# VISION-SJTU/UniDefense

Measured on AMD Instinct MI355X. Metric: images/sec fwd+bwd (256x256, EffNet-b4), higher is better.
Workload: dtype f32

## Files before the change

include/unidefense_hip.h:

```cpp
#ifndef UNIDEFENSE_HIP_H
#define UNIDEFENSE_HIP_H
#include <stdint.h>

#ifdef __cplusplus
extern "C" {
#endif

#define UD_EINVAL (-1000)

typedef void* ud_stream_t;

typedef struct {
    int N, Hin, Win, Cin, Hout, Wout, KH, KW, stride, pad_t, pad_l, transposed;
} ud_conv_geom;

typedef struct {
    const float* A; const float* B; float* C;
    int M, N, K;
    long lda, ldb, ldc;
    int a_mode, b_mode, out_mode, split_k;
    int batch; long strideA, strideB, strideC;
    ud_conv_geom g;
    double* stat_sum; double* stat_sumsq;
    int half_mask;
    int tile_cfg;
    long slice_stride;
} ud_gemm_desc;
int ud_gemm(const ud_gemm_desc* d, ud_stream_t stream);
int ud_sum_slices(const float* ws, float* out, int slices, long total, long slice_stride, int accumulate,
                  ud_stream_t stream);
int ud_gemm_stats_slots(const ud_gemm_desc* d);
int ud_stat_slots_fold(const double* slot_sum, const double* slot_sumsq, int slots, int N, double* acc_sum,
                       double* acc_sumsq, ud_stream_t stream);
int ud_gemm_set_path(int path);
int ud_gemm_get_path(void);
int ud_gemm_query_path(const ud_gemm_desc* d);

typedef struct {
    const uint16_t* A; const uint16_t* B; float* C;
    int M, N, K;
    long a_panel, a_plane, b_panel, b_plane;
    int a_npanel, b_npanel;
    long ldc;
    int a_mode, b_mode, out_mode, split_k;
    double* stat_sum; double* stat_sumsq;
    int tile_cfg;
    long slice_stride;
    int prec;
    const float* a_inv_scale; const float* b_inv_scale;
    int a_scale_stride, b_scale_stride;
    int c_half;
} ud_gemm_p3_desc;
int ud_gemm_p3(const ud_gemm_p3_desc* d, ud_stream_t stream);
int ud_gemm_p3_pair(const ud_gemm_p3_desc* nn, const ud_gemm_p3_desc* tn, ud_stream_t stream);
int ud_planes_from_half(const void* x, long R, int C, long ld, uint16_t* planes, long panel_stride, float* inv_scale,
                        ud_stream_t stream);
int ud_split_planes(const float* x, long R, int C, long ld, uint16_t* planes, long panel_stride, long plane_stride,
                    ud_stream_t stream);
int ud_split_planes_h2(const float* x, long R, int C, long ld, uint16_t* planes, long panel_stride, long plane_stride,
                       float* inv_scale, ud_stream_t stream);
int ud_absmax(const float* x, long R, int C, long ld, uint32_t* absmax, ud_stream_t stream);
int ud_split_planes_h2t(const float* x, long R, int C, long ld, uint16_t* planes, long panel_stride, long plane_stride,
                        const uint32_t* absmax, float* inv_scale, ud_stream_t stream);
typedef struct {
    const float* x; uint16_t* out; float* inv_scale;
    long R, ld, panel, plane;
    int C, amax_block0, amax_blocks, split_block0, split_bx, pad_;
} ud_split_item;
int ud_split_planes_h2t_multi(const ud_split_item* items_dev, int n, uint32_t* slots, int amax_blocks_total,
                              int split_blocks_total, ud_stream_t stream);

int ud_im2col_planes(const float* x, const ud_conv_geom* g, uint16_t* planes, long panel_stride, long plane_stride,
                     const uint32_t* absmax, float* inv_scale, ud_stream_t stream);
int ud_col2im(const float* dcol, const ud_conv_geom* g, float* dx, ud_stream_t stream);

typedef struct {
    const float* src;
    float* dst;
    int A, B, KH, KW, mode, block0;
} ud_layout_item;
int ud_weight_layouts_multi(const ud_layout_item* items_dev, int n, int blocks_total, ud_stream_t stream);

int ud_reduce_ws_doubles(int G, int R, int C);
int ud_norm_stats(const float* x, int G, int R, int C, float eps, double* ws, float* mean, float* invstd,
                  float* var_out, float momentum, float* running_mean, float* running_var, ud_stream_t stream);
int ud_syncbn_combine(const float* gathered, int world, int C, long rows_per_rank, float eps, float momentum,
                      float* running_mean, float* running_var, float* mean, float* invstd, ud_stream_t stream);
int ud_norm_apply_fwd(const float* x, int G, int R, int C, const float* mean, const float* invstd,
                      const float* gamma, const float* beta, int act, float* y, ud_stream_t stream);
int ud_norm_bwd(const float* x, const float* dy, int G, int R, int C, const float* mean, const float* invstd,
                const float* gamma, const float* beta, int act, double* ws, float* s1, float* s2, float* dgamma,
                float* dbeta, float* dx, ud_stream_t stream);
int ud_norm_bwd_apply(const float* x, const float* dy, int G, int R, int C, const float* mean,
                      const float* invstd, const float* gamma, const float* beta, const float* s1,
                      const float* s2, float inv_count, int act, float* dx, ud_stream_t stream);
int ud_group_colsum(const float* x, int G, int R, int C, float scale, double* ws, float* out, ud_stream_t stream);
int ud_group_coldot(const float* a, const float* b, int G, int R, int C, float scale, double* ws, float* out,
                    ud_stream_t stream);
int ud_bcast_rows(const float* g, float scale, float* out, int N, int HW, int C, ud_stream_t stream);

int ud_dwconv_fwd(const void* x, const float* wt, void* y, int N, int H, int W, int C, int Ho, int Wo, int K,
    int stride, int pad_t, int pad_l, int f16, ud_stream_t stream);
int ud_dwconv_bwd_data(const void* dy, const float* wt, const void* add, void* dx, int N, int H, int W, int C,
    int Ho, int Wo, int K, int stride, int pad_t, int pad_l, int f16, ud_stream_t stream);
int ud_dwconv_bwd_weight_parts(int C, int chunks);
int ud_dw_weights_tapmajor(const void* table, int layers, long max_elems, float* dst, ud_stream_t stream);
int ud_dwconv_bwd_weight(const float* x, const float* dy, float* dwt, float* part, int chunks, int N,
                         int H, int W, int C, int Ho, int Wo, int K, int stride, int pad_t, int pad_l,
                         ud_stream_t stream);

int ud_rfft2(const void* x, void* Y, int N, int S, int C, float scale, float w_interior, int f16, ud_stream_t
    stream);
int ud_irfft2(const void* Y, void* x, int N, int S, int C, float scale, float w_interior, int f16, ud_stream_t
    stream);
int ud_fft32_set_wave(int mode);

int ud_fc_fwd(const float* x, const float* W, const float* b, float* y, int N, int I, int O, int act_in,
              ud_stream_t stream);
int ud_fc_bwd(const float* dy, const float* W, const float* x, float* dx, float* dW, float* db, int N,
              int I, int O, int act_in, ud_stream_t stream);

int ud_se_scale_fwd(const float* x, const float* s, float* y, int N, int HW, int C, ud_stream_t stream);
int ud_se_scale_bwd(const float* dy, const float* s, const float* dpool, float* dx, int N, int HW, int C,
                    ud_stream_t stream);
int ud_sigmoid_grad_mul(const float* s, float* v, long n, ud_stream_t stream);

int ud_sfmix_blocks(int N, int Ho, int Wo, int C);
int ud_sfmix_fwd(const void* spat, const void* freq, const float* alpha, void* y, int N, int Ho, int Wo, int C,
    int pool, int f16, ud_stream_t stream);
int ud_sfmix_bwd(const void* spat, const void* freq, const float* alpha, const void* dy, void* dspat, void*
    dfreq, double* part, float* dalpha, int N, int Ho, int Wo, int C, int pool, int f16, ud_stream_t stream);
int ud_sfmix_pool_bwd(const void* dy, void* dfreq, int N, int Ho, int Wo, int C, int f16, ud_stream_t stream);
int ud_gate_mix_blocks(long total);
int ud_gate_mix_fwd(const float* p, const float* q, const float* alpha, float* y, long total,
                    ud_stream_t stream);
int ud_gate_mix_bwd(const float* p, const float* q, const float* alpha, const float* dy, float* dp, float* dq,
                    double* part, float* dalpha, long total, ud_stream_t stream);

int ud_residual_fwd(const float* x, const float* skip, const float* keep, float inv_keep, float* out,
                    long total, long per_sample, ud_stream_t stream);
int ud_axpby(const void* a, float alpha, const void* b, float beta, void* out, long total, int f16, ud_stream_t
    stream);
int ud_mask_scale(const float* x, const float* mask, float scale, float* out, long total,
                  ud_stream_t stream);
int ud_absdiff(const float* a, const float* b, float* out, long total, ud_stream_t stream);

int ud_pix_to_planes(const float* in, float* out, int N, int C, int HW, int mode, ud_stream_t stream);
int ud_planes_to_pix(const float* in, const float* aux, float* out, int N, int C, int HW, int mode,
                     ud_stream_t stream);
int ud_bilinear_fwd(const float* x, float* y, int P, int Hi, int Wi, int Ho, int Wo, ud_stream_t stream);
int ud_bilinear_bwd(const float* dy, float* dx, int P, int Hi, int Wi, int Ho, int Wo, ud_stream_t stream);
int ud_l1_chunks(long per_sample);
int ud_l1_fwd(const float* a, const float* b, float* part, float* out, int N, long per_sample, float scale,
              ud_stream_t stream);
int ud_l1_bwd(const float* a, const float* b, const float* g, float scale, int accumulate, float* da, int N,
              long per_sample, ud_stream_t stream);

int ud_dynfilter_fwd(const float* proj, const float* diff, const float* w2, const float* x, float* pre,
                     int* argmax, float* mask, float* out, int M, int C, int D, int Cx, ud_stream_t stream);
int ud_dynfilter_bwd(const float* dout, const float* dmask_ext, const float* x, const float* mask,
                     const int* argmax, const float* w2, float* dx, float* dlogit, float* dproj, int M,
                     int C, int Cx, ud_stream_t stream);

int ud_avgpool_fwd(const float* x, float* y, int N, int Ho, int Wo, int C, int k, ud_stream_t stream);
int ud_avgpool_bwd(const float* dy, float* dx, int N, int Ho, int Wo, int C, int k, ud_stream_t stream);
int ud_adaptive_avgpool_fwd(const float* x, float* y, int N, int H, int W, int Ho, int Wo, int C, ud_stream_t stream);
int ud_adaptive_avgpool_bwd(const float* dy, float* dx, int N, int H, int W, int Ho, int Wo, int C, ud_stream_t stream);
int ud_maxpool3s2_fwd(const float* x, float* y, unsigned char* arg, int N, int H, int W, int C,
                      ud_stream_t stream);
int ud_maxpool3s2_bwd(const float* dy, const unsigned char* arg, float* dx, int N, int H, int W, int C,
                      ud_stream_t stream);
int ud_add_act_fwd(const float* a, const float* b, int act, float* y, long total, ud_stream_t stream);
int ud_relu_bwd(const float* dy, const float* y, float* g, long total, ud_stream_t stream);
int ud_copy_cols(float* narrow, float* wide, long M, int Cn, int Cw, int off, int dir, ud_stream_t stream);

int ud_aw_triplet(const float* feat, int N, int D, int n_real, float* loss, float* dfeat, float* ws,
                  ud_stream_t stream);

typedef struct {
    const float* feat[3]; float* dfeat[3]; int D[3]; int nfeat;
    const float* cls; const long long* tgt; float* dcls; int N, C, R, F;
    const float* fm; float* dfm; int nfm; const float* sm; float* dsm; int nsm;
    const float* spatial; float* dspatial; const float* freq; float* dfreq;
    float w_cls, w_fm, w_sm, w_trip, w_rec, w_freq;
    float* vals;
    float* ws;
} ud_loss_tail;
int ud_loss_tail_ws_floats(int N, int n_real, int nfeat);
int ud_loss_tail_run(const ud_loss_tail* t, ud_stream_t stream);

int ud_conv_small_supported(int Cin, int Cout, int KH, int KW);
int ud_conv_small(const ud_conv_geom* g, const float* x, const float* wmat, float* y, int Cout, ud_stream_t stream);
int ud_conv_small_wgrad_supported(int Cin, int Ma, int KH, int KW);
long ud_conv_small_wgrad_ws_floats(int Cin, int Ma);
int ud_conv_small_wgrad(const ud_conv_geom* g, const float* a, const float* x, float* part, float* out, int Ma,
                        ud_stream_t stream);

int ud_conv_mfma_mode(const ud_conv_geom* g);
int ud_conv_mfma_supported(int Cin, int Cout, int mode);
int ud_conv_mfma(const ud_conv_geom* g, const float* x, const float* wmat, float* y, int Cout, ud_stream_t stream);
int ud_conv_mfma_wgrad_supported(int Cin, int Ma, int mode);
long ud_conv_mfma_wgrad_ws_floats(int Cin, int Ma);
int ud_conv_mfma_wgrad(const ud_conv_geom* g, const float* a, const float* x, float* part, float* out, int Ma,
                       ud_stream_t stream);

int ud_stem_dgrad_supported(int Cin, int Cout, int KH, int KW, int stride);
int ud_stem_dgrad(const ud_conv_geom* g, const float* dy, const float* w, float* dx, int Cout, int accumulate,
                  ud_stream_t stream);
int ud_absdiff_bwd(const float* a, const float* b, const float* g, float* da, float* db, long total, ud_stream_t stream);
int ud_outer(const float* u, const float* v, float* out, long M, int D, ud_stream_t stream);

int ud_attack_step_linf(float* x_adv, const float* x0, const float* g, long total, float step, float eps, float lo, float hi,
                        ud_stream_t stream);
long ud_sample_sumsq_ws_bytes(int N, long per);
int ud_sample_sumsq(const float* a, const float* b, int N, long per, double* out, double* ws, long ws_bytes,
                    ud_stream_t stream);
int ud_attack_step_l2(float* x_adv, const float* g, const double* gss, int N, long per, float step, ud_stream_t stream);
int ud_attack_project_l2(float* x_adv, const float* x0, const double* dss, int N, long per, float eps, float lo, float hi,
                         ud_stream_t stream);

#define UD_APGD_MAX_CHECKPOINTS 16
#define UD_APGD_I_K 0
#define UD_APGD_I_CNT 1
#define UD_APGD_I_HALVED 2
#define UD_APGD_I_IMPROVED 3
#define UD_APGD_I_RESET 4
#define UD_APGD_F_PREV 0
#define UD_APGD_F_BEST 1
#define UD_APGD_F_CKPT 2
#define UD_APGD_F_ETA 3
#define UD_APGD_F_A 4
int ud_apgd_control(const float* f, int* ist, float* fst, float* history, int N, int steps, const int* ck_w,
                    const int* ck_thr, int n_ck, float eta0, float alpha, int closing, ud_stream_t stream);
int ud_apgd_update_linf(float* x, float* x_prev, float* x_best, float* g_best, const float* x0, const float* g, const int* ist,
                        const float* fst, int N, long per, float eps, float lo, float hi, ud_stream_t stream);
int ud_apgd_keep(float* dst, const float* src, const int* flag, int N, long per, ud_stream_t stream);
int ud_apgd_step_l2(float* x, float* z, float* x_best, float* g_best, double* gss_best, const float* g, const double* gss,
                    const int* ist, const float* fst, int N, long per, ud_stream_t stream);
int ud_apgd_combine_l2(float* x, float* x_prev, const float* z, const float* fst, int N, long per, ud_stream_t stream);
int ud_apgd_project_l2(float* x, const float* x0, const double* dss, const float* fst, int N, long per, float eps, float lo,
                       float hi, ud_stream_t stream);

#define UD_FMN_CHUNK 4096
#define UD_FMN_PARTS 4
#define UD_FMN_P_GSS 0
// ... 281 lines not shown
    float inv_hw, void* dz, double* s1, double* s2, double* ws, int G, int R, int C, int f16, ud_stream_t
    stream);
int ud_coldot_bn_se(const void* dy, const void* x, const ud_bn_ref* bn, int G, int R, int C, double* out, int f16,
                    ud_stream_t stream);
int ud_se_bwd_b_bn(const double* ds1_acc, const float* s1, const float* Wr, const double* pool, float pool_scale,
                   float* dpool, float* dWr, float* dbr, const float* s2, const double* dots, float inv_hw, double* bs1,
                   double* bs2, int N, int C, int Cs, ud_stream_t stream);
int ud_normbwd_apply_se(const void* x, const void* dc, const ud_bn_ref* bn, const float* s, const float* dpool, float inv_hw,
                        const double* s1, const double* s2, const double* s1_local, const double* s2_local, int G, int R,
                        int C, void* dx, float* dgamma, float* dbeta, int f16, uint32_t* absmax, ud_stream_t stream);
int ud_normbwd_apply_mix_se(const void* x, const void* dc, const ud_bn_ref* bn, const float* s, const float* dpool,
                            float inv_hw, const double* s1, const double* s2, const double* s1_local,
                            const double* s2_local, const void* diff, int G, int R, int C, void* dd, double* dalpha_acc,
                            float* dgamma, float* dbeta, double* energy, int f16, ud_stream_t stream);
long ud_coldot_bn_eval_ws_doubles(int G, int R, int C);
int ud_coldot_bn_eval(const void* dy, const void* x, const ud_bn_ref* bn, int G, int R, int C, double* out, double* ws,
                      int f16, ud_stream_t stream);
int ud_se_scale_bwd_bn_eval(const void* dc, const void* x, const ud_bn_ref* bn, const float* s, const float* dpool,
                            float inv_hw, void* dd, int G, int R, int C, int f16, ud_stream_t stream);
int ud_bn_eval_bwd(const void* dy, const void* x, const ud_bn_ref* bn, void* dx, int G, int R, int C, int f16,
                   ud_stream_t stream);
int ud_normbwd_apply_mix(const void* x, const void* dz, const ud_bn_ref* bn, const double* s1, const double* s2,
    const double* s1_local, const double* s2_local, const void* diff, int G, int R, int C, void* dd,
    double* dalpha_acc, float* dgamma, float* dbeta, double* energy, int f16, ud_stream_t stream);
int ud_gate_grad_from_acc(const double* acc, const float* alpha, float* out, ud_stream_t stream);
int ud_bn_apply(const void* x, const ud_bn_ref* bn, void* y, int G, int R, int C, int f16, ud_stream_t stream);
int ud_dwconv_bwd_data_bn(const void* dy, const float* gate_alpha, int gate_mode, const float* wt, const void*
    add, const void* x, const ud_bn_ref* bn, void* dz, double* s1, double* s2, double* ws, int N, int H, int W,
    int C, int Ho, int Wo, int K, int stride, int pad_t, int pad_l, int f16, ud_stream_t stream);
long ud_dwconv_bwd_data_bn_ws_doubles(int N, int H, int W, int C, int stride);
int ud_dwconv_bwd_data_ex(const void* dy, const float* gate_alpha, int gate_mode, const float* wt, const void*
    add, void* dx, int N, int H, int W, int C, int Ho, int Wo, int K, int stride, int pad_t, int pad_l, int f16,
    ud_stream_t stream);
int ud_dwconv_bwd_weight_ex(const void* x, const void* dy, const float* gate_alpha, int gate_mode, float* dwt,
    float* part, int chunks, int N, int H, int W, int C, int Ho, int Wo, int K, int stride, int pad_t, int
    pad_l, int f16, ud_stream_t stream);
int ud_rfft2_ex(const void* x, void* Y, int N, int S, int C, float scale, float w_interior, const ud_bn_ref* bn,
    void* act_out, const float* gate_alpha, int gate_mode, const double* gate_acc, float* gate_grad, int f16,
    uint32_t* absmax, ud_stream_t stream);
int ud_rfft2_ex_planes(const void* x, uint16_t* planes, long panel_stride, long plane_stride, float* inv_scale, float bound_pre,
                       const double* energy, int N, int S, int C, float scale, float w_interior, const ud_bn_ref* bn,
                       void* act_out, const float* gate_alpha, int gate_mode, const double* gate_acc, float* gate_grad,
                       const float* dw_wt, void* dw_out, int dw_k, ud_stream_t stream);
int ud_irfft2_mix(const void* Y, void* y, int N, int S, int C, float scale, float w_interior, const void* spat,
    const float* alpha, void* diff_out, double* sum, double* sumsq, int f16, ud_stream_t stream);

long ud_fft2_two_pass_ws_floats(int N, int S, int C);
int ud_rfft2_two_pass(const void* x, void* Y, float* ws, int N, int S, int C, float scale, float w_interior,
    const ud_bn_ref* bn, void* act_out, const float* gate_alpha, int gate_mode, const double* gate_acc,
    float* gate_grad, int f16, uint32_t* absmax, ud_stream_t stream);
int ud_irfft2_two_pass(const void* Y, void* y, float* ws, int N, int S, int C, float scale, float w_interior,
    const void* spat, const float* alpha, void* freq_out, double* sum, double* sumsq, int f16, ud_stream_t stream);

int ud_adamw_chunk_elems(void);
int ud_adamw_multi(const void* table, const void* chunk_map, int n_chunks, const float* lr, const float* wd, int n_groups,
                   double beta1, double beta2, double eps, int amsgrad, int maximize, const float* grad_scale,
                   const float* found_inf, const int* step_in, int* step_out, ud_stream_t stream);

int ud_multi_add(void* const* dst, const void* const* src, const long* numel, int n, ud_stream_t stream);

long ud_dwtile_ws_doubles(int N, int Ho, int Wo, int C);
int ud_dwtile(const void* src, const ud_bn_ref* bn_in, const float* wt, void* out, int N, int Hs, int Ws, int C, int Ho,
              int Wo, int K, int P_t, int P_l, int flip, const float* gate_alpha, int gate_mode, const void* add,
              const void* xbn, const ud_bn_ref* bn_out, int epi, double* s1, double* s2, double* ws, int stride,
              int f16, ud_stream_t stream);
long ud_dwtile_wgrad_part_rows(int N, int Ho, int Wo);
int ud_dwtile_wgrad(const void* src, const ud_bn_ref* bn_in, const void* dy, const float* gate_alpha, int gate_mode,
                    float* dwt, float* part, long part_rows, int N, int Hs, int Ws, int C, int Ho, int Wo, int K, int P_t,
                    int P_l, int stride, int f16, ud_stream_t stream);
int ud_dwtile_bwd(const void* dy, const void* x, const ud_bn_ref* bn, const float* wt, const float* gate_alpha, int gate_mode,
                  const void* add, void* dz, float* dwt, float* wpart, long part_rows, double* s1, double* s2, double* ws,
                  int N, int H, int W, int C, int K, int P_t, int P_l, int f16, ud_stream_t stream);
int ud_dwtile_dgrad_eval(const void* dy, const float* wt, const float* gate_alpha, int gate_mode, const void* add,
                         const void* xbn, const ud_bn_ref* bn, void* dx, int N, int H, int W, int C, int Ho, int Wo, int K,
                         int pad_t, int pad_l, int stride, int f16, ud_stream_t stream);
int ud_dwtile_wgrad_finalize(const float* part, int nparts, int K, int C, const float* gate_alpha, int gate_mode, float* dwt,
                             ud_stream_t stream);
#define UD_FOLD_DW 0
#define UD_FOLD_F32 1
#define UD_FOLD_PJ 2
#define UD_FOLD_F64 3
#define UD_FOLD_GROUP 4
#define UD_FOLD_LAYOUT 5
typedef struct {
    const float* part;
    float* dst;
    const float* aux;
    const double* s1l;
    const double* s2l;
    float* dgamma;
    float* dbeta;
    int kind, nparts, n, p0, p1, p2;
} ud_wgrad_fold;
int ud_param_fold_multi(const ud_wgrad_fold* items, int n, ud_stream_t stream);
int ud_rfft2_ex_plane_half(const void* x, uint16_t* plane, long panel_stride, float* inv_scale, int N, int S, int C, float scale,
                           float w_interior, const ud_bn_ref* bn, void* act_out, const float* gate_alpha, int gate_mode,
                           const double* gate_acc, float* gate_grad, const float* dw_wt, void* dw_out, int dw_k,
                           ud_stream_t stream);
int ud_irfft2_dwbwd(const void* Y, int N, int S, int C, float scale, float w_interior, const void* dd, const void* x,
                    const ud_bn_ref* bn, const float* wt, int K, const float* gate_alpha, int gate_mode, void* dz, double* s1,
                    double* s2, double* s3, float* wpart, int f16, ud_stream_t stream);

long ud_rfft2_planes_ws_floats(long P, int S);
int ud_rfft2_planes(const float* x, float* Y, float* ws, long P, int S, float scale, ud_stream_t stream);
int ud_rfft2_planes_adjoint(const float* dY, float* dx, float* ws, long P, int S, float scale, ud_stream_t stream);

long ud_xchg_bytes(int world, int max_doubles, int slots);
int ud_xchg_create(int world, int max_doubles, int slots, void** base, char* handle);
int ud_xchg_open(const char* handle, void** ptr);
int ud_xchg_close(void* ptr);
int ud_xchg_destroy(void* base);
int ud_xchg_allreduce(double* acc, int n, void* const* peers, int rank, int world, int max_doubles, int slots,
                      unsigned long long* seq_counter, int* err, long timeout_ms, double* local_out, ud_stream_t stream);

#ifdef __cplusplus
}
#endif
#endif
```

unidefense_amd/csrc/fused.hip:

```cpp
#include "bnref.h"

namespace {

struct Rows {
    int r, r_end;
    long idx, step;
};
__device__ __forceinline__ Rows rows_of(const RedGeom& q, int ri, int c4) {
    Rows w;
    const int g = blockIdx.z, p = blockIdx.x;
    const int r_begin = p * q.rows_per_chunk;
    w.r_end = r_begin + q.rows_per_chunk;
    if (w.r_end > q.R) w.r_end = q.R;
    w.step = (long)q.rpi * q.C4;
    w.r = r_begin + ri;
    w.idx = (long)g * q.R * q.C4 + (long)w.r * q.C4 + c4;
    return w;
}

__device__ __forceinline__ bool is_updater(int ri) { return blockIdx.x == 0 && blockIdx.z == 0 && ri == 0; }

template <int NQ>
__device__ __forceinline__ void red_out(const RedGeom& q, int ri, bool active, int c4, double (&v)[8], double* a1,
                                        double* a2, double* part, bool per_group) {
// ... 959 lines not shown
                if (add) da += add4[o];
                if (BN) {
                    const f32x4 a = x4[o];
#pragma unroll
                    for (int e = 0; e < 4; ++e) {
                        const float xh = (a[e] - cb.mu[e]) * cb.is[e];
                        float g = da[e];
                        if (bn.act) g *= ud_act_grad_fast(cb.ga[e] * xh + cb.be[e], bn.act);
                        g = ud_rounded<T>(g);
                        da[e] = g;
                        v[e] += (double)g;
                        v[4 + e] += (double)g * (double)xh;
                    }
                }
                o4.st(o, da);
            }
        }
    }
    if (BN) red_out<8>(q, ri, active, c4, v, s1, s2, part, false);
}

template <typename T, int K, int S>
__global__ __launch_bounds__(NT) void dw_bwd_weight_rows_ex(DwGeom q, int C, int rows_per_group, const T* __restrict__ x,
                                      const T* __restrict__ dy, float* __restrict__ part) {
    constexpr int CPL = sizeof(T) == 2 ? 2 : 1;
    typedef T VT __attribute__((ext_vector_type(CPL == 2 ? 2 : 1)));
    typedef float VF __attribute__((ext_vector_type(CPL == 2 ? 2 : 1)));
    const int c = (blockIdx.y * blockDim.x + threadIdx.x) * CPL;
    if (c >= C) return;
    const int p = blockIdx.x;
    const int rows_total = q.N * q.Ho;
    const int row0 = p * rows_per_group;
    int row1 = row0 + rows_per_group;
    if (row1 > rows_total) row1 = rows_total;
    const VF zero = {};
    auto ld = [](const T* ptr) { return __builtin_convertvector(*reinterpret_cast<const VT*>(ptr), VF); };
    VF acc[K * K];
#pragma unroll
    for (int i = 0; i < K * K; ++i) acc[i] = zero;
    for (int row = row0; row < row1; ++row) {
        const int n = row / q.Ho, ho = row % q.Ho;
        const int ih0 = ho * S - q.pad_t;
        const T* xr[K];
        bool vh[K];
#pragma unroll
        for (int kh = 0; kh < K; ++kh) {
            const int ih = ih0 + kh;
            vh[kh] = (ih >= 0) && (ih < q.H);
            xr[kh] = x + (((long)n * q.H + (vh[kh] ? ih : 0)) * q.W) * C + c;
        }
        VF w[K][K];
#pragma unroll
        for (int kh = 0; kh < K; ++kh)
#pragma unroll
            for (int kw = 0; kw < K; ++kw) {
                const int iw = kw - q.pad_l;
                w[kh][kw] = (vh[kh] && iw >= 0 && iw < q.W) ? ld(xr[kh] + (long)iw * C) : zero;
            }
        const T* dyr = dy + ((long)row * q.Wo) * C + c;
#pragma unroll 4
        for (int wo = 0; wo < q.Wo; ++wo) {
            const VF g = ld(dyr + (long)wo * C);
#pragma unroll
            for (int kh = 0; kh < K; ++kh)
#pragma unroll
                for (int kw = 0; kw < K; ++kw) acc[kh * K + kw] += g * w[kh][kw];
#pragma unroll
            for (int kh = 0; kh < K; ++kh) {
#pragma unroll
                for (int kw = 0; kw + S < K; ++kw) w[kh][kw] = w[kh][kw + S];
#pragma unroll
                for (int j = 0; j < S; ++j) {
                    const int iw = (wo + 1) * S - q.pad_l + (K - S) + j;
                    w[kh][K - S + j] = (vh[kh] && iw >= 0 && iw < q.W) ? ld(xr[kh] + (long)iw * C) : zero;
                }
            }
        }
    }
    float* out = part + (long)p * (K * K) * C + c;
#pragma unroll
    for (int i = 0; i < K * K; ++i) *reinterpret_cast<VF*>(out + (long)i * C) = acc[i];
}

__global__ __launch_bounds__(NT) void dw_bwd_weight_finalize_ex(int nparts, int KK, int C, const float* __restrict__ part,
                                                                const float* __restrict__ gate_alpha, int gate_mode,
                                                                float* __restrict__ dw) {
    const int KKC = KK * C;
    __shared__ double sm[16][16][4];
    const int lane = threadIdx.x & 15, sl = threadIdx.x >> 4;
    const int i = (blockIdx.x * 16 + lane) * 4;
    double a[4] = {0.0, 0.0, 0.0, 0.0};
    if (i < KKC) {
        const f32x4* p4 = reinterpret_cast<const f32x4*>(part + i);
        const long step = (long)KKC / 4;
        int p = sl;
        for (; p + 48 < nparts; p += 64) {
            const f32x4 v0 = p4[(long)p * step], v1 = p4[(long)(p + 16) * step];
            const f32x4 v2 = p4[(long)(p + 32) * step], v3 = p4[(long)(p + 48) * step];
#pragma unroll
            for (int e = 0; e < 4; ++e) a[e] += ((double)v0[e] + (double)v1[e]) + ((double)v2[e] + (double)v3[e]);
        }
        for (; p < nparts; p += 16) {
            const f32x4 v = p4[(long)p * step];
#pragma unroll
            for (int e = 0; e < 4; ++e) a[e] += (double)v[e];
        }
    }
#pragma unroll
    for (int e = 0; e < 4; ++e) sm[sl][lane][e] = a[e];
    __syncthreads();
    if (sl < 4 && i < KKC) {
        double t = 0.0;
#pragma unroll
        for (int k = 0; k < 16; ++k) t += sm[k][lane][sl];
        const int o = i + sl, tap = o / C, c = o % C;
        dw[(long)c * KK + tap] = (float)(t * (double)gate_factor(gate_alpha, gate_mode));
    }
}

inline bool dw_geom_ok(const DwGeom& q, int K) {
    return q.N > 0 && q.H > 0 && q.W > 0 && q.C4 > 0 && q.Ho > 0 && q.Wo > 0 && (q.stride == 1 || q.stride == 2) &&
           (K == 3 || K == 5);
}

inline bool shape_ok(int G, int R, int C) { return G >= 1 && R >= 1 && C >= 4 && C % 4 == 0; }

struct RedPlan {
    RedGeom q;
    bool use_part;
};
inline RedPlan plan_reduce(int G, int R, int C, bool per_group, const double* ws, int min_rows = 8,
                           int row_elems = 1) {
    constexpr int lim = 64;
    constexpr long big_elems = 1L << 20;
    RedGeom qa = make_geom_ex(G, R, C, 1024, lim, min_rows);
    const long contrib = per_group ? qa.P : (long)qa.G * qa.P;
    const bool big = !per_group && (long)G * R * row_elems * (C / 4) >= big_elems;
    if ((contrib <= lim && !big) || !ws) return RedPlan{qa, false};
    return RedPlan{make_geom_ex(G, R, C, 2048, 512, min_rows), true};
}
inline int finish_reduce(const RedPlan& pl, int nq, bool per_group, int C, const double* ws, double* a1, double* a2,
                         hipStream_t s) {
    if (!pl.use_part) return 0;
    const int G = per_group ? pl.q.G : 1;
    const int P = per_group ? pl.q.P : pl.q.G * pl.q.P;
    hipLaunchKernelGGL(partials_to_acc, dim3(ud_cdiv((long)G * C, 8)), dim3(NT), 0, s, nq, G, C, P, ws, a1, a2);
    UD_LAUNCH_CHECK();
    return 0;
}
inline RedGeom geom_ew(int G, int R, int C, int min_rows = 4) { return make_geom_ex(G, R, C, 2048, 4096, min_rows, 128); }

}

extern "C" {

long ud_fused_reduce_ws_doubles(int G, int R, int C, int per_group, int min_rows) {
    if (!shape_ok(G, R, C) || min_rows < 1) return UD_EINVAL;
    static double dummy;
    RedPlan pl = plan_reduce(G, R, C, per_group != 0, &dummy, min_rows);
    return pl.use_part ? 2L * pl.q.G * pl.q.P * C : 0;
}

int ud_stat_slots_fold(const double* slot_sum, const double* slot_sumsq, int slots, int N, double* acc_sum,
                       double* acc_sumsq, ud_stream_t stream) {
    if (!slot_sum || !slot_sumsq || slots < 1 || N < 1 || !acc_sum || !acc_sumsq) return UD_EINVAL;
    hipStream_t s = (hipStream_t)stream;
    if (slot_sumsq == slot_sum + (long)slots * N) {
        hipLaunchKernelGGL(partials_to_acc, dim3(ud_cdiv(N, 8)), dim3(NT), 0, s, 2, 1, N, slots, slot_sum, acc_sum, acc_sumsq);
    } else {
        hipLaunchKernelGGL(partials_to_acc, dim3(ud_cdiv(N, 8)), dim3(NT), 0, s, 1, 1, N, slots, slot_sum, acc_sum, nullptr);
        hipLaunchKernelGGL(partials_to_acc, dim3(ud_cdiv(N, 8)), dim3(NT), 0, s, 1, 1, N, slots, slot_sumsq, acc_sumsq, nullptr);
    }
    UD_LAUNCH_CHECK();
    return 0;
}

int ud_colstats(const void* x, int G, int R, int C, double* sum, double* sumsq, double* ws, int f16,
                ud_stream_t stream) {
    if (!shape_ok(G, R, C) || !x || !sum || !sumsq) return UD_EINVAL;
    hipStream_t s = (hipStream_t)stream;
    RedPlan pl = plan_reduce(G, R, C, G != 1, ws);
    UD_STORAGE_DISPATCH(f16, hipLaunchKernelGGL(colstats_kernel<T>, red_grid(pl.q), dim3(NT), 0, s, pl.q, (const T*)x, sum,
                                                sumsq, pl.use_part ? ws : nullptr));
    UD_LAUNCH_CHECK();
    return finish_reduce(pl, 2, G != 1, C, ws, sum, sumsq, s);
}

int ud_colsum_bn(const void* x, const ud_bn_ref* bn, int G, int R, int C, double* out, double* ws, int f16,
                 ud_stream_t stream) {
    if (!shape_ok(G, R, C) || !x || !bn || !out) return UD_EINVAL;
    hipStream_t s = (hipStream_t)stream;
    RedPlan pl = plan_reduce(G, R, C, true, ws);
    UD_STORAGE_DISPATCH(f16, hipLaunchKernelGGL((colsum_bn_kernel<T, false>), red_grid(pl.q), dim3(NT), 0, s, pl.q,
                                                (const T*)x, (const T*)nullptr, *bn, out, pl.use_part ? ws : nullptr,
                                                (uint32_t*)nullptr));
    UD_LAUNCH_CHECK();
    return finish_reduce(pl, 1, true, C, ws, out, nullptr, s);
}

int ud_colsum_bn_amax(const void* x, const ud_bn_ref* bn, int G, int R, int C, double* out, double* ws, uint32_t* absmax,
                      ud_stream_t stream) {
    if (!shape_ok(G, R, C) || !x || !bn || !out || !absmax) return UD_EINVAL;
// ... 326 lines not shown

int ud_bn_eval_bwd(const void* dy, const void* x, const ud_bn_ref* bn, void* dx, int G, int R, int C, int f16,
                   ud_stream_t stream) {
    if (!ud_bn_eval_form(bn) || bn->G != 1) return UD_EINVAL;
    if (!shape_ok(G, R, C) || !dy || !dx || (bn->act && !x) || bn->act < 0 || bn->act > 2) return UD_EINVAL;
    RedGeom q = geom_ew(G, R, C);
    UD_STORAGE_DISPATCH(f16, hipLaunchKernelGGL(bn_eval_bwd_kernel<T>, red_grid(q), dim3(NT), 0, (hipStream_t)stream, q,
                                                (const T*)dy, (const T*)x, *bn, (T*)dx));
    UD_LAUNCH_CHECK();
    return 0;
}

static long dw_bwd_items(int N, int H, int W, int stride) {
    return stride == 1 ? (long)N * H * ((W + TW - 1) / TW) : (long)N * H * W;
}
long ud_dwconv_bwd_data_bn_ws_doubles(int N, int H, int W, int C, int stride) {
    const long items = dw_bwd_items(N, H, W, stride);
    if (items < 1 || items > 0x7fffffffL || C % 4 || C < 4) return UD_EINVAL;
    static double dummy;
    RedPlan pl = plan_reduce(1, (int)items, C, false, &dummy, stride == 1 ? 1 : 4, stride == 1 ? TW : 1);
    return pl.use_part ? 2L * pl.q.G * pl.q.P * C : 0;
}

}

template <typename T>
static int dw_bwd_data_launch(const T* dy, const float* gate_alpha, int gate_mode, const float* wt, const T* add,
                              const T* x, const ud_bn_ref* bn, T* out, double* s1, double* s2, double* ws, int N,
                              int H, int W, int C, int Ho, int Wo, int K, int stride, int pad_t, int pad_l, hipStream_t s) {
    if (C % 4 || !dy || !wt || !out) return UD_EINVAL;
    DwGeom d{N, H, W, C / 4, Ho, Wo, stride, pad_t, pad_l};
    if (!dw_geom_ok(d, K)) return UD_EINVAL;
    const bool strip = stride == 1;
    const long items = dw_bwd_items(N, H, W, stride);
    if (items > 0x7fffffffL) return UD_EINVAL;
    ud_bn_ref none{};
    const bool has_bn = bn != nullptr;
    if (has_bn && (!x || !s1 || !s2 || bn->G != 1)) return UD_EINVAL;
    RedPlan pl{make_geom_ex(1, (int)items, C, 2048, 8192, strip ? 1 : 4), false};
    if (has_bn) pl = plan_reduce(1, (int)items, C, false, ws, strip ? 1 : 4, strip ? TW : 1);
    const RedGeom& q = pl.q;
    double* part = pl.use_part ? ws : nullptr;
    const ud_bn_ref& b = has_bn ? *bn : none;
#define UD_DW_BWD(KK, ST, BB)                                                                                        \
    hipLaunchKernelGGL((dw_bwd_data_ex_kernel<T, KK, ST, BB>), red_grid(q), dim3(NT), 0, s, q, d, dy, gate_alpha,    \
                       gate_mode, wt, add, x, b, out, s1, s2, part)
    if (K == 3) {
        if (strip) { if (has_bn) UD_DW_BWD(3, true, true); else UD_DW_BWD(3, true, false); }
        else { if (has_bn) UD_DW_BWD(3, false, true); else UD_DW_BWD(3, false, false); }
    } else {
        if (strip) { if (has_bn) UD_DW_BWD(5, true, true); else UD_DW_BWD(5, true, false); }
        else { if (has_bn) UD_DW_BWD(5, false, true); else UD_DW_BWD(5, false, false); }
    }
#undef UD_DW_BWD
    UD_LAUNCH_CHECK();
    return has_bn ? finish_reduce(pl, 2, false, C, ws, s1, s2, s) : 0;
}

extern "C" {

int ud_dwconv_bwd_data_bn(const void* dy, const float* gate_alpha, int gate_mode, const float* wt, const void* add,
                          const void* x, const ud_bn_ref* bn, void* dz, double* s1, double* s2, double* ws, int N,
                          int H, int W, int C, int Ho, int Wo, int K, int stride, int pad_t, int pad_l, int f16,
                          ud_stream_t stream) {
    if (ud_bn_eval_form(bn)) return UD_EINVAL;
    if (!bn) return UD_EINVAL;
    UD_STORAGE_DISPATCH(f16, return dw_bwd_data_launch<T>((const T*)dy, gate_alpha, gate_mode, wt, (const T*)add,
                                                          (const T*)x, bn, (T*)dz, s1, s2, ws, N, H, W, C, Ho, Wo, K,
                                                          stride, pad_t, pad_l, (hipStream_t)stream));
}

int ud_dwconv_bwd_data_ex(const void* dy, const float* gate_alpha, int gate_mode, const float* wt, const void* add,
                          void* dx, int N, int H, int W, int C, int Ho, int Wo, int K, int stride, int pad_t,
                          int pad_l, int f16, ud_stream_t stream) {
    UD_STORAGE_DISPATCH(f16, return dw_bwd_data_launch<T>((const T*)dy, gate_alpha, gate_mode, wt, (const T*)add,
                                                          (const T*)nullptr, nullptr, (T*)dx, nullptr, nullptr, nullptr,
                                                          N, H, W, C, Ho, Wo, K, stride, pad_t, pad_l,
                                                          (hipStream_t)stream));
}

int ud_dwconv_bwd_weight_ex(const void* x, const void* dy, const float* gate_alpha, int gate_mode, float* dwt,
                            float* part, int chunks, int N, int H, int W, int C, int Ho, int Wo, int K, int stride,
                            int pad_t, int pad_l, int f16, ud_stream_t stream) {
    if (C % 4 || chunks < 1 || !x || !dy || !dwt || !part) return UD_EINVAL;
    DwGeom q{N, H, W, C / 4, Ho, Wo, stride, pad_t, pad_l};
    if (!dw_geom_ok(q, K)) return UD_EINVAL;
    hipStream_t s = (hipStream_t)stream;
    const int rows_total = N * Ho;
    if (chunks > rows_total) return UD_EINVAL;
    const int rpg = (rows_total + chunks - 1) / chunks;
    const int lanes = f16 ? C / 2 : C;
    int bt = ((lanes < NT ? lanes : NT) + 63) / 64 * 64;
    dim3 grid((unsigned)chunks, (unsigned)ud_cdiv(lanes, bt), 1);
#define UD_DW_WG(KK, SS)                                                                                              \
    UD_STORAGE_DISPATCH(f16, hipLaunchKernelGGL((dw_bwd_weight_rows_ex<T, KK, SS>), grid, dim3(bt), 0, s, q, C, rpg,         \
                                                (const T*)x, (const T*)dy, part))
    if (K == 3 && stride == 1) UD_DW_WG(3, 1);
    else if (K == 3) UD_DW_WG(3, 2);
    else if (stride == 1) UD_DW_WG(5, 1);
    else UD_DW_WG(5, 2);
#undef UD_DW_WG
    UD_LAUNCH_CHECK();
    const int KKC = K * K * C;
    hipLaunchKernelGGL(dw_bwd_weight_finalize_ex, dim3(ud_cdiv(KKC, 64)), dim3(NT), 0, s, chunks, K * K, C, part,
                       gate_alpha, gate_mode, dwt);
    UD_LAUNCH_CHECK();
    return 0;
}

}
```

unidefense_amd/csrc/misc.hip:

```cpp
#include "ud_common.h"

namespace {

constexpr int NT = 256;

inline int ew_blocks(long total, int cap = 8192) {
    long b = (total + NT - 1) / NT;
    if (b > cap) b = cap;
    if (b < 1) b = 1;
    return (int)b;
}

__device__ __forceinline__ float act_in_f(float x, int act) { return act == 1 ? ud_swish(x) : x; }

__global__ __launch_bounds__(NT) void fc_fwd(const float* __restrict__ x, const float* __restrict__ W,
                                             const float* __restrict__ b, float* __restrict__ y, int N, int I, int O,
                                             int act_in) {
    const int wave = (blockIdx.x * NT + threadIdx.x) >> 6, lane = threadIdx.x & 63;
    if (wave >= N * O) return;
    const int n = wave / O, o = wave % O;
    float acc = 0.f;
#pragma unroll 4
    for (int i = lane; i < I; i += 64) acc += act_in_f(x[(long)n * I + i], act_in) * W[(long)o * I + i];
    acc = ud_wave_sum(acc);
// ... 120 lines not shown
    const long b = ((n * H + 2 * ho) * W + 2 * wo) * C4 + c4;
    f32x4 v = f4[b] + f4[b + C4] + f4[b + (long)W * C4] + f4[b + (long)W * C4 + C4];
    return v * 0.25f;
}

template <typename T>
__global__ __launch_bounds__(NT) void sfmix_fwd(long total4, int Ho, int Wo, int C4, int pool,
                                                const T* __restrict__ spat, const T* __restrict__ freq,
                                                const float* __restrict__ alpha, T* __restrict__ y) {
    const float a = ud_sigmoid(alpha[0]);
    const In4<T> s4{spat}, f4{freq};
    const Out4<T> y4{y};
    for (long e = (long)blockIdx.x * NT + threadIdx.x; e < total4; e += (long)gridDim.x * NT) {
        int c4 = (int)(e % C4);
        long pix = e / C4;
        int wo = (int)(pix % Wo);
        long t = pix / Wo;
        int ho = (int)(t % Ho);
        long n = t / Ho;
        f32x4 fp = pooled_freq(f4, pool, n, ho, wo, Ho, Wo, C4, c4);
        y4.st(e, s4[e] * (1.f - a) + fp * a);
    }
}

template <typename T>
__global__ __launch_bounds__(NT) void sfmix_bwd(long total4, int Ho, int Wo, int C4, int pool,
                                                const T* __restrict__ spat, const T* __restrict__ freq,
                                                const float* __restrict__ alpha, const T* __restrict__ dy,
                                                T* __restrict__ dspat, T* __restrict__ dfreq,
                                                double* __restrict__ part) {
    const float a = ud_sigmoid(alpha[0]);
    const In4<T> s4{spat}, f4{freq}, d4{dy};
    const Out4<T> ds4{dspat}, df4{dfreq};
    double acc = 0.0;
    for (long e = (long)blockIdx.x * NT + threadIdx.x; e < total4; e += (long)gridDim.x * NT) {
        int c4 = (int)(e % C4);
        long pix = e / C4;
        int wo = (int)(pix % Wo);
        long t = pix / Wo;
        int ho = (int)(t % Ho);
        long n = t / Ho;
        f32x4 fp = pooled_freq(f4, pool, n, ho, wo, Ho, Wo, C4, c4);
        f32x4 d = d4[e], s = s4[e];
        ds4.st(e, d * (1.f - a));
        if (!pool) {
            df4.st(e, d * a);
        } else {
            const int H = Ho * 2, W = Wo * 2;
            const long b = ((n * H + 2 * ho) * W + 2 * wo) * C4 + c4;
            f32x4 g = d * (0.25f * a);
            df4.st(b, g); df4.st(b + C4, g); df4.st(b + (long)W * C4, g); df4.st(b + (long)W * C4 + C4, g);
        }
#pragma unroll
        for (int k = 0; k < 4; ++k) acc += (double)d[k] * ((double)fp[k] - (double)s[k]);
    }
    __shared__ double sm[NT / 64];
    acc = ud_wave_sum_d(acc);
    if ((threadIdx.x & 63) == 0) sm[threadIdx.x >> 6] = acc;
    __syncthreads();
    if (threadIdx.x == 0) {
        double tot = 0.0;
        for (int i = 0; i < NT / 64; ++i) tot += sm[i];
        part[blockIdx.x] = tot;
    }
}

template <typename T>
__global__ __launch_bounds__(NT) void sfmix_pool_bwd(long total4, int H, int W, int C4, const T* __restrict__ dy,
                                                     T* __restrict__ dfreq) {
    const In4<T> d4{dy};
    const Out4<T> o4{dfreq};
    const int Ho = H / 2, Wo = W / 2;
    for (long e = (long)blockIdx.x * NT + threadIdx.x; e < total4; e += (long)gridDim.x * NT) {
        const int c4 = (int)(e % C4);
        const long pix = e / C4;
        const int w = (int)(pix % W);
        const long t = pix / W;
        const int h = (int)(t % H);
        const long n = t / H;
        o4.st(e, d4[((n * Ho + h / 2) * Wo + w / 2) * C4 + c4] * 0.25f);
    }
}

__global__ __launch_bounds__(NT) void gate_grad_finalize(int n, const double* __restrict__ part,
                                                         const float* __restrict__ alpha, float* __restrict__ out) {
    double acc = 0.0;
    for (int i = threadIdx.x; i < n; i += NT) acc += part[i];
    __shared__ double sm[NT / 64];
    acc = ud_wave_sum_d(acc);
    if ((threadIdx.x & 63) == 0) sm[threadIdx.x >> 6] = acc;
    __syncthreads();
    if (threadIdx.x == 0) {
        double tot = 0.0;
        for (int i = 0; i < NT / 64; ++i) tot += sm[i];
        double a = 1.0 / (1.0 + exp(-(double)alpha[0]));
        out[0] = (float)(tot * a * (1.0 - a));
    }
}


__global__ __launch_bounds__(NT) void residual_fwd(long total4, long per_sample4, const float* __restrict__ x,
                                                   const float* __restrict__ skip, const float* __restrict__ keep,
                                                   float inv_keep, float* __restrict__ out) {
    const f32x4* x4 = reinterpret_cast<const f32x4*>(x);
    const f32x4* k4 = reinterpret_cast<const f32x4*>(skip);
    f32x4* o4 = reinterpret_cast<f32x4*>(out);
    for (long e = (long)blockIdx.x * NT + threadIdx.x; e < total4; e += (long)gridDim.x * NT) {
        float sc = keep ? keep[e / per_sample4] * inv_keep : 1.f;
        f32x4 v = x4[e] * sc;
        if (skip) v += k4[e];
        o4[e] = v;
    }
}

template <typename T>
__global__ __launch_bounds__(NT) void axpby(long total, const T* __restrict__ a, float alpha,
                                            const T* __restrict__ b, float beta, T* __restrict__ out) {
    for (long e = (long)blockIdx.x * NT + threadIdx.x; e < total; e += (long)gridDim.x * NT) {
        float v = (float)a[e] * alpha;
        if (b) v += (float)b[e] * beta;
        out[e] = (T)v;
    }
}

__global__ __launch_bounds__(NT) void sum_slices(long total4, int slices, long stride4, const float* __restrict__ ws,
                                                 float* __restrict__ out, int accumulate) {
    const f32x4* w4 = reinterpret_cast<const f32x4*>(ws);
    f32x4* o4 = reinterpret_cast<f32x4*>(out);
    for (long e = (long)blockIdx.x * NT + threadIdx.x; e < total4; e += (long)gridDim.x * NT) {
        f32x4 v = accumulate ? o4[e] : f32x4{0, 0, 0, 0};
        for (int s = 0; s < slices; ++s) v += w4[(long)s * stride4 + e];
        o4[e] = v;
    }
}

__global__ __launch_bounds__(NT) void mask_scale(long total, const float* __restrict__ x, const float* __restrict__ m,
                                                 float scale, float* __restrict__ out) {
    for (long e = (long)blockIdx.x * NT + threadIdx.x; e < total; e += (long)gridDim.x * NT)
        out[e] = x[e] * m[e] * scale;
}

__global__ __launch_bounds__(NT) void bcast_rows(long total4, int HW, int C4, const float* __restrict__ g, float scale,
                                                 float* __restrict__ out) {
    const f32x4* g4 = reinterpret_cast<const f32x4*>(g);
    f32x4* o4 = reinterpret_cast<f32x4*>(out);
    for (long e = (long)blockIdx.x * NT + threadIdx.x; e < total4; e += (long)gridDim.x * NT) {
        long row = e / C4;
        int c4 = (int)(e - row * C4);
        long n = row / HW;
        o4[e] = g4[n * C4 + c4] * scale;
    }
}

__global__ __launch_bounds__(NT) void absdiff(long total, const float* __restrict__ a, const float* __restrict__ b,
                                              float* __restrict__ out) {
    for (long e = (long)blockIdx.x * NT + threadIdx.x; e < total; e += (long)gridDim.x * NT)
        out[e] = fabsf(a[e] - (b ? b[e] : 0.f));
}

__global__ __launch_bounds__(NT) void gate_mix_fwd(long total, const float* __restrict__ p, const float* __restrict__ q,
                                                   const float* __restrict__ alpha, float* __restrict__ y) {
    const float a = ud_sigmoid(alpha[0]);
    for (long e = (long)blockIdx.x * NT + threadIdx.x; e < total; e += (long)gridDim.x * NT)
        y[e] = (1.f - a) * p[e] + a * q[e];
}

__global__ __launch_bounds__(NT) void gate_mix_bwd(long total, const float* __restrict__ p, const float* __restrict__ q,
                                                   const float* __restrict__ alpha, const float* __restrict__ dy,
                                                   float* __restrict__ dp, float* __restrict__ dq,
                                                   double* __restrict__ part) {
    const float a = ud_sigmoid(alpha[0]);
    double acc = 0.0;
    for (long e = (long)blockIdx.x * NT + threadIdx.x; e < total; e += (long)gridDim.x * NT) {
        float d = dy[e];
        dp[e] = (1.f - a) * d;
        dq[e] = a * d;
        acc += (double)d * ((double)q[e] - (double)p[e]);
    }
    __shared__ double sm[NT / 64];
    acc = ud_wave_sum_d(acc);
// ... 93 lines not shown
            if (wh == 0.f) continue;
            float row = 0.f;
            for (int wo = wo_lo; wo <= wo_hi; ++wo) row += bil_weight(wo, w, Wi, Wo) * g[(long)ho * Wo + wo];
            acc += wh * row;
        }
        dx[e] = acc;
    }
}

__global__ __launch_bounds__(NT) void l1_partial(long per_sample, const float* __restrict__ a,
                                                 const float* __restrict__ b, float* __restrict__ part) {
    const long n = blockIdx.y;
    const float* pa = a + n * per_sample;
    const float* pb = b ? b + n * per_sample : nullptr;
    float acc = 0.f;
    for (long e = (long)blockIdx.x * NT + threadIdx.x; e < per_sample; e += (long)gridDim.x * NT)
        acc += fabsf(pa[e] - (pb ? pb[e] : 0.f));
    __shared__ float sm[NT / 64];
    acc = ud_wave_sum(acc);
    if ((threadIdx.x & 63) == 0) sm[threadIdx.x >> 6] = acc;
    __syncthreads();
    if (threadIdx.x == 0) {
        float tot = 0.f;
        for (int i = 0; i < NT / 64; ++i) tot += sm[i];
        part[n * gridDim.x + blockIdx.x] = tot;
    }
}

__global__ void l1_finalize(int N, int P, const float* __restrict__ part, float scale, float* __restrict__ out) {
    int n = blockIdx.x * blockDim.x + threadIdx.x;
    if (n >= N) return;
    float a = 0.f;
    for (int p = 0; p < P; ++p) a += part[(long)n * P + p];
    out[n] = a * scale;
}

__global__ __launch_bounds__(NT) void l1_bwd(long total, long per_sample, const float* __restrict__ a,
                                             const float* __restrict__ b, const float* __restrict__ g, float scale,
                                             int accumulate, float* __restrict__ da) {
    for (long e = (long)blockIdx.x * NT + threadIdx.x; e < total; e += (long)gridDim.x * NT) {
        float d = a[e] - (b ? b[e] : 0.f);
        float s = (d > 0.f) ? 1.f : ((d < 0.f) ? -1.f : 0.f);
        float v = g[e / per_sample] * scale * s;
        da[e] = accumulate ? da[e] + v : v;
    }
}

__global__ __launch_bounds__(NT) void dynfilter_fwd(int M, int C, int D, int Cx, const float* __restrict__ proj,
                                                    const float* __restrict__ diff, const float* __restrict__ w2,
                                                    const float* __restrict__ x, float* __restrict__ pre,
                                                    int* __restrict__ argmax, float* __restrict__ mask,
                                                    float* __restrict__ out) {
    const int m = (blockIdx.x * NT + threadIdx.x) >> 6, lane = threadIdx.x & 63;
    if (m >= M) return;
    const float* pr = proj + (long)m * C;
    float s = 0.f, mx = -INFINITY;
    int am = 0x7fffffff;
    for (int c = lane; c < C; c += 64) {
        float v = pr[c];
        s += v;
        if (v > mx) { mx = v; am = c; }
    }
    s = ud_wave_sum(s);
#pragma unroll
    for (int o = 32; o > 0; o >>= 1) {
        float omx = __shfl_xor(mx, o, 64);
        int oam = __shfl_xor(am, o, 64);
        if (omx > mx || (omx == mx && oam < am)) { mx = omx; am = oam; }
    }
    const float mean = s / (float)C;
    float logit = w2[0] * mean + w2[1] * mx;
    for (int j = 0; j < D; ++j) logit += w2[2 + j] * diff[(long)m * D + j];
    const float mk = ud_sigmoid(logit);
    if (lane == 0) {
        pre[(long)m * (2 + D)] = mean;
        pre[(long)m * (2 + D) + 1] = mx;
        for (int j = 0; j < D; ++j) pre[(long)m * (2 + D) + 2 + j] = diff[(long)m * D + j];
        argmax[m] = am;
        mask[m] = mk;
    }
    for (int c = lane; c < Cx; c += 64) out[(long)m * Cx + c] = mk * x[(long)m * Cx + c];
}

__global__ __launch_bounds__(NT) void dynfilter_bwd(int M, int C, int Cx, const float* __restrict__ dout,
                                                    const float* __restrict__ dmask_ext, const float* __restrict__ x,
                                                    const float* __restrict__ mask, const int* __restrict__ argmax,
                                                    const float* __restrict__ w2, float* __restrict__ dx,
                                                    float* __restrict__ dlogit, float* __restrict__ dproj) {
    const int m = (blockIdx.x * NT + threadIdx.x) >> 6, lane = threadIdx.x & 63;
    if (m >= M) return;
    const float mk = mask[m];
    float acc = 0.f;
    for (int c = lane; c < Cx; c += 64) {
        float d = dout[(long)m * Cx + c];
        acc += d * x[(long)m * Cx + c];
        dx[(long)m * Cx + c] = mk * d;
    }
    acc = ud_wave_sum(acc);
    const float dm = acc + (dmask_ext ? dmask_ext[m] : 0.f);
    const float dl = dm * mk * (1.f - mk);
    if (lane == 0) dlogit[m] = dl;
    const float gm = dl * w2[0] / (float)C, gx = dl * w2[1];
    const int am = argmax[m];
    for (int c = lane; c < C; c += 64) dproj[(long)m * C + c] = gm + ((c == am) ? gx : 0.f);
}

struct DwWtEntry { const float* src; long C, KK, dst_off; };
__global__ __launch_bounds__(NT) void dw_wt_tapmajor(const DwWtEntry* __restrict__ tab, float* __restrict__ dst) {
    const DwWtEntry e = tab[blockIdx.y];
    const long n = e.C * e.KK;
    const long i = (long)blockIdx.x * NT + threadIdx.x;
    if (i >= n) return;
    const long tap = i / e.C, c = i - tap * e.C;
    dst[e.dst_off + i] = e.src[c * e.KK + tap];
}

__global__ __launch_bounds__(NT) void weight_layouts_kernel(const ud_layout_item* __restrict__ items, int n) {
    int lo = 0, hi = n - 1;
    while (lo < hi) {
        const int mid = (lo + hi + 1) >> 1;
        if (items[mid].block0 <= (int)blockIdx.x) lo = mid;
        else hi = mid - 1;
    }
    const ud_layout_item it = items[lo];
    const long e = (long)(blockIdx.x - it.block0) * NT + threadIdx.x;
    const long total = (long)it.A * it.B * it.KH * it.KW;
    if (e >= total) return;
    const int taps = it.KH * it.KW;
    const int inner = it.mode == 0 ? it.B : it.A;
    const int col = (int)(e % inner);
    const int tap = (int)((e / inner) % taps);
    const int row = (int)(e / ((long)inner * taps));
    const int a = it.mode == 0 ? row : col, b = it.mode == 0 ? col : row;
    const int st = it.mode == 1 ? taps - 1 - tap : tap;
    it.dst[e] = it.src[((long)a * it.B + b) * taps + st];
}

}

extern "C" {

int ud_weight_layouts_multi(const ud_layout_item* items_dev, int n, int blocks_total, ud_stream_t stream) {
    if (!items_dev || n < 1 || blocks_total < n) return UD_EINVAL;
    hipLaunchKernelGGL(weight_layouts_kernel, dim3((unsigned)blocks_total), dim3(NT), 0, (hipStream_t)stream, items_dev, n);
    UD_LAUNCH_CHECK();
    return 0;
}


int ud_fc_fwd(const float* x, const float* W, const float* b, float* y, int N, int I, int O, int act_in,
              ud_stream_t stream) {
    if (I <= 128 && O >= 256) {
        hipLaunchKernelGGL(fc_fwd_wide, dim3(ud_cdiv(O, NT), N), dim3(NT), 0, (hipStream_t)stream, x, W, b, y, N, I, O,
                           act_in);
        UD_LAUNCH_CHECK();
        return 0;
    }
    long waves = (long)N * O;
    hipLaunchKernelGGL(fc_fwd, dim3(ud_cdiv(waves * 64, NT)), dim3(NT), 0, (hipStream_t)stream, x, W, b, y, N, I, O,
                       act_in);
    UD_LAUNCH_CHECK();
    return 0;
}

int ud_fc_bwd(const float* dy, const float* W, const float* x, float* dx, float* dW, float* db, int N, int I, int O,
              int act_in, ud_stream_t stream) {
    hipStream_t s = (hipStream_t)stream;
    if (dx) {
        if (O >= 256)
            hipLaunchKernelGGL(fc_bwd_x_wave, dim3(ud_cdiv((long)N * I * 64, NT)), dim3(NT), 0, s, dy, W, x, dx, N, I,
                               O, act_in);
        else
            hipLaunchKernelGGL(fc_bwd_x, dim3(ud_cdiv((long)N * I, NT)), dim3(NT), 0, s, dy, W, x, dx, N, I, O, act_in);
        UD_LAUNCH_CHECK();
    }
    if (dW) {
        hipLaunchKernelGGL(fc_bwd_w, dim3(ud_cdiv((long)O * I, NT)), dim3(NT), 0, s, dy, x, dW, db, N, I, O, act_in);
        UD_LAUNCH_CHECK();
    }
    return 0;
}

int ud_se_scale_fwd(const float* x, const float* s, float* y, int N, int HW, int C, ud_stream_t stream) {
    if (C % 4) return UD_EINVAL;
    long total4 = (long)N * HW * (C / 4);
    hipLaunchKernelGGL(se_scale_fwd, dim3(ew_blocks(total4)), dim3(NT), 0, (hipStream_t)stream, total4, HW, C / 4, x, s,
                       y);
    UD_LAUNCH_CHECK();
    return 0;
}

int ud_se_scale_bwd(const float* dy, const float* s, const float* dpool, float* dx, int N, int HW, int C,
                    ud_stream_t stream) {
    if (C % 4) return UD_EINVAL;
    long total4 = (long)N * HW * (C / 4);
    hipLaunchKernelGGL(se_scale_bwd, dim3(ew_blocks(total4)), dim3(NT), 0, (hipStream_t)stream, total4, HW, C / 4, dy,
                       s, dpool, 1.f / (float)HW, dx);
    UD_LAUNCH_CHECK();
    return 0;
}

int ud_sigmoid_grad_mul(const float* s, float* v, long n, ud_stream_t stream) {
    hipLaunchKernelGGL(sigmoid_grad_mul, dim3(ud_cdiv(n, 256)), dim3(256), 0, (hipStream_t)stream, n, s, v);
    UD_LAUNCH_CHECK();
    return 0;
}

int ud_sfmix_blocks(int N, int Ho, int Wo, int C) { return ew_blocks((long)N * Ho * Wo * (C / 4), 1024); }

int ud_sfmix_fwd(const void* spat, const void* freq, const float* alpha, void* y, int N, int Ho, int Wo, int C,
                 int pool, int f16, ud_stream_t stream) {
    if (C % 4) return UD_EINVAL;
    long total4 = (long)N * Ho * Wo * (C / 4);
    UD_STORAGE_DISPATCH(f16, hipLaunchKernelGGL(sfmix_fwd<T>, dim3(ew_blocks(total4)), dim3(NT), 0, (hipStream_t)stream,
                                                total4, Ho, Wo, C / 4, pool, (const T*)spat, (const T*)freq, alpha,
                                                (T*)y));
    UD_LAUNCH_CHECK();
    return 0;
}

int ud_sfmix_bwd(const void* spat, const void* freq, const float* alpha, const void* dy, void* dspat, void* dfreq,
                 double* part, float* dalpha, int N, int Ho, int Wo, int C, int pool, int f16, ud_stream_t stream) {
    if (C % 4) return UD_EINVAL;
    hipStream_t s = (hipStream_t)stream;
    long total4 = (long)N * Ho * Wo * (C / 4);
    int nb = ew_blocks(total4, 1024);
    UD_STORAGE_DISPATCH(f16, hipLaunchKernelGGL(sfmix_bwd<T>, dim3(nb), dim3(NT), 0, s, total4, Ho, Wo, C / 4, pool,
                                                (const T*)spat, (const T*)freq, alpha, (const T*)dy, (T*)dspat,
                                                (T*)dfreq, part));
    UD_LAUNCH_CHECK();
    hipLaunchKernelGGL(gate_grad_finalize, dim3(1), dim3(NT), 0, s, nb, part, alpha, dalpha);
    UD_LAUNCH_CHECK();
    return 0;
}

int ud_sfmix_pool_bwd(const void* dy, void* dfreq, int N, int Ho, int Wo, int C, int f16, ud_stream_t stream) {
    if (N < 1 || Ho < 1 || Wo < 1 || C < 4 || C % 4 || !dy || !dfreq) return UD_EINVAL;
    const long total4 = (long)N * Ho * Wo * 4 * (C / 4);
    UD_STORAGE_DISPATCH(f16, hipLaunchKernelGGL(sfmix_pool_bwd<T>, dim3(ew_blocks(total4)), dim3(NT), 0, (hipStream_t)stream,
                                                total4, 2 * Ho, 2 * Wo, C / 4, (const T*)dy, (T*)dfreq));
    UD_LAUNCH_CHECK();
    return 0;
}

int ud_gate_mix_blocks(long total) { return ew_blocks(total, 1024); }

int ud_gate_mix_fwd(const float* p, const float* q, const float* alpha, float* y, long total, ud_stream_t stream) {
    hipLaunchKernelGGL(gate_mix_fwd, dim3(ew_blocks(total)), dim3(NT), 0, (hipStream_t)stream, total, p, q, alpha, y);
    UD_LAUNCH_CHECK();
    return 0;
}

int ud_gate_mix_bwd(const float* p, const float* q, const float* alpha, const float* dy, float* dp, float* dq,
                    double* part, float* dalpha, long total, ud_stream_t stream) {
    hipStream_t s = (hipStream_t)stream;
    int nb = ew_blocks(total, 1024);
    hipLaunchKernelGGL(gate_mix_bwd, dim3(nb), dim3(NT), 0, s, total, p, q, alpha, dy, dp, dq, part);
    UD_LAUNCH_CHECK();
    hipLaunchKernelGGL(gate_grad_finalize, dim3(1), dim3(NT), 0, s, nb, part, alpha, dalpha);
    UD_LAUNCH_CHECK();
    return 0;
}

int ud_residual_fwd(const float* x, const float* skip, const float* keep, float inv_keep, float* out, long total,
                    long per_sample, ud_stream_t stream) {
    if (total % 4 || per_sample % 4) return UD_EINVAL;
    hipLaunchKernelGGL(residual_fwd, dim3(ew_blocks(total / 4)), dim3(NT), 0, (hipStream_t)stream, total / 4,
                       per_sample / 4, x, skip, keep, inv_keep, out);
    UD_LAUNCH_CHECK();
    return 0;
}

int ud_axpby(const void* a, float alpha, const void* b, float beta, void* out, long total, int f16, ud_stream_t stream) {
    UD_STORAGE_DISPATCH(f16, hipLaunchKernelGGL(axpby<T>, dim3(ew_blocks(total)), dim3(NT), 0, (hipStream_t)stream, total,
                                                (const T*)a, alpha, (const T*)b, beta, (T*)out));
    UD_LAUNCH_CHECK();
    return 0;
}

int ud_sum_slices(const float* ws, float* out, int slices, long total, long slice_stride, int accumulate,
                  ud_stream_t stream) {
    if (!ws || !out || slices < 1 || total < 4 || total % 4 || slice_stride % 4 || slice_stride < total) return UD_EINVAL;
    hipLaunchKernelGGL(sum_slices, dim3(ew_blocks(total / 4)), dim3(NT), 0, (hipStream_t)stream, total / 4, slices,
                       slice_stride / 4, ws, out, accumulate);
    UD_LAUNCH_CHECK();
    return 0;
}

int ud_mask_scale(const float* x, const float* mask, float scale, float* out, long total, ud_stream_t stream) {
    hipLaunchKernelGGL(mask_scale, dim3(ew_blocks(total)), dim3(NT), 0, (hipStream_t)stream, total, x, mask, scale,
                       out);
    UD_LAUNCH_CHECK();
    return 0;
}

int ud_bcast_rows(const float* g, float scale, float* out, int N, int HW, int C, ud_stream_t stream) {
    if (C % 4) return UD_EINVAL;
    long total4 = (long)N * HW * (C / 4);
    hipLaunchKernelGGL(bcast_rows, dim3(ew_blocks(total4)), dim3(NT), 0, (hipStream_t)stream, total4, HW, C / 4, g,
                       scale, out);
    UD_LAUNCH_CHECK();
    return 0;
}

int ud_absdiff(const float* a, const float* b, float* out, long total, ud_stream_t stream) {
    hipLaunchKernelGGL(absdiff, dim3(ew_blocks(total)), dim3(NT), 0, (hipStream_t)stream, total, a, b, out);
    UD_LAUNCH_CHECK();
    return 0;
}

int ud_pix_to_planes(const float* in, float* out, int N, int C, int HW, int mode, ud_stream_t stream) {
    long total = (long)N * C * HW;
    hipLaunchKernelGGL(pix_to_planes, dim3(ew_blocks(total)), dim3(NT), 0, (hipStream_t)stream, total, C, HW, in, out,
                       mode);
    UD_LAUNCH_CHECK();
    return 0;
}

int ud_planes_to_pix(const float* in, const float* aux, float* out, int N, int C, int HW, int mode,
                     ud_stream_t stream) {
    long total = (long)N * C * HW;
    hipLaunchKernelGGL(planes_to_pix, dim3(ew_blocks(total)), dim3(NT), 0, (hipStream_t)stream, total, C, HW, in, aux,
                       out, mode);
    UD_LAUNCH_CHECK();
    return 0;
}

int ud_bilinear_fwd(const float* x, float* y, int P, int Hi, int Wi, int Ho, int Wo, ud_stream_t stream) {
    long total = (long)P * Ho * Wo;
    hipLaunchKernelGGL(bilinear_fwd, dim3(ew_blocks(total)), dim3(NT), 0, (hipStream_t)stream, total, Hi, Wi, Ho, Wo, x,
                       y);
    UD_LAUNCH_CHECK();
    return 0;
}

int ud_bilinear_bwd(const float* dy, float* dx, int P, int Hi, int Wi, int Ho, int Wo, ud_stream_t stream) {
    hipStream_t s = (hipStream_t)stream;
    long total = (long)P * Hi * Wi;
    hipLaunchKernelGGL(bilinear_bwd, dim3(ew_blocks(total)), dim3(NT), 0, s, total, Hi, Wi, Ho, Wo, dy, dx);
    UD_LAUNCH_CHECK();
    return 0;
}

int ud_l1_chunks(long per_sample) { return ew_blocks(per_sample, 64); }

int ud_l1_fwd(const float* a, const float* b, float* part, float* out, int N, long per_sample, float scale,
              ud_stream_t stream) {
    hipStream_t s = (hipStream_t)stream;
    int P = ew_blocks(per_sample, 64);
    hipLaunchKernelGGL(l1_partial, dim3(P, N), dim3(NT), 0, s, per_sample, a, b, part);
    UD_LAUNCH_CHECK();
    hipLaunchKernelGGL(l1_finalize, dim3(ud_cdiv(N, 64)), dim3(64), 0, s, N, P, part, scale, out);
    UD_LAUNCH_CHECK();
    return 0;
}

int ud_l1_bwd(const float* a, const float* b, const float* g, float scale, int accumulate, float* da, int N,
              long per_sample, ud_stream_t stream) {
    long total = (long)N * per_sample;
    hipLaunchKernelGGL(l1_bwd, dim3(ew_blocks(total)), dim3(NT), 0, (hipStream_t)stream, total, per_sample, a, b, g,
                       scale, accumulate, da);
    UD_LAUNCH_CHECK();
    return 0;
}

int ud_dynfilter_fwd(const float* proj, const float* diff, const float* w2, const float* x, float* pre, int* argmax,
                     float* mask, float* out, int M, int C, int D, int Cx, ud_stream_t stream) {
    hipLaunchKernelGGL(dynfilter_fwd, dim3(ud_cdiv((long)M * 64, NT)), dim3(NT), 0, (hipStream_t)stream, M, C, D, Cx,
                       proj, diff, w2, x, pre, argmax, mask, out);
    UD_LAUNCH_CHECK();
    return 0;
}

int ud_dynfilter_bwd(const float* dout, const float* dmask_ext, const float* x, const float* mask, const int* argmax,
                     const float* w2, float* dx, float* dlogit, float* dproj, int M, int C, int Cx,
                     ud_stream_t stream) {
    hipLaunchKernelGGL(dynfilter_bwd, dim3(ud_cdiv((long)M * 64, NT)), dim3(NT), 0, (hipStream_t)stream, M, C, Cx, dout,
                       dmask_ext, x, mask, argmax, w2, dx, dlogit, dproj);
    UD_LAUNCH_CHECK();
    return 0;
}

int ud_dw_weights_tapmajor(const void* table, int layers, long max_elems, float* dst, ud_stream_t stream) {
    if (layers < 1 || max_elems < 1 || !table || !dst) return UD_EINVAL;
    hipLaunchKernelGGL(dw_wt_tapmajor, dim3((unsigned)ud_cdiv(max_elems, NT), (unsigned)layers), dim3(NT), 0,
                       (hipStream_t)stream, reinterpret_cast<const DwWtEntry*>(table), dst);
    UD_LAUNCH_CHECK();
    return 0;
}

}
```

unidefense_amd/csrc/norm.hip:

```cpp
#include "colgeom.h"

namespace {

constexpr int NT = UD_COL_NT;

enum { RED_STATS = 0, RED_NORMBWD = 1, RED_SUM = 2, RED_DOT = 3 };

template <int MODE>
__device__ __forceinline__ void accumulate(const f32x4& a, const f32x4& b, const f32x4& mu, const f32x4& is,
                                           const f32x4& ga, const f32x4& be, int act, double (&v)[8]) {
#pragma unroll
    for (int e = 0; e < 4; ++e) {
        if (MODE == RED_STATS) {
            double d = (double)a[e];
            v[e] += d;
            v[4 + e] += d * d;
        } else if (MODE == RED_NORMBWD) {
            float xh = (a[e] - mu[e]) * is[e];
            float dz = b[e];
            if (act) dz *= ud_act_grad(ga[e] * xh + be[e], act);
            v[e] += (double)dz;
            v[4 + e] += (double)dz * (double)xh;
        } else if (MODE == RED_SUM) {
            v[e] += (double)a[e];
        } else {
            v[e] += (double)a[e] * (double)b[e];
        }
    }
}

template <int MODE>
__global__ __launch_bounds__(NT) void colreduce_partial(RedGeom q, const float* __restrict__ x,
                                                        const float* __restrict__ y2,
                                                        const float* __restrict__ mean,
                                                        const float* __restrict__ invstd,
                                                        const float* __restrict__ gamma, const float* __restrict__ beta,
                                                        int act, double* __restrict__ part1, double* __restrict__ part2) {
    constexpr bool HAS_Y = (MODE == RED_NORMBWD || MODE == RED_DOT);
    constexpr int NQ = (MODE == RED_STATS || MODE == RED_NORMBWD) ? 8 : 4;
    int ri, c4;
    bool active = thread_coords(q, ri, c4);
    const int g = blockIdx.z, p = blockIdx.x;
    const int r_begin = p * q.rows_per_chunk;
    int r_end = r_begin + q.rows_per_chunk;
    if (r_end > q.R) r_end = q.R;
    const long gbase = (long)g * q.R * q.C4;
    const f32x4* x4 = reinterpret_cast<const f32x4*>(x);
    const f32x4* y4 = reinterpret_cast<const f32x4*>(y2);
    double v[8] = {0, 0, 0, 0, 0, 0, 0, 0};
    if (active) {
        f32x4 mu = {0, 0, 0, 0}, is = mu, ga = mu, be = mu;
        if (MODE == RED_NORMBWD) {
            mu = reinterpret_cast<const f32x4*>(mean)[(long)g * q.C4 + c4];
            is = reinterpret_cast<const f32x4*>(invstd)[(long)g * q.C4 + c4];
            ga = reinterpret_cast<const f32x4*>(gamma)[c4];
            be = reinterpret_cast<const f32x4*>(beta)[c4];
        }
        const long step = (long)q.rpi * q.C4;
        int r = r_begin + ri;
        long idx = gbase + (long)r * q.C4 + c4;
        for (; r + 3 * q.rpi < r_end; r += 4 * q.rpi, idx += 4 * step) {
            f32x4 a0 = x4[idx], a1 = x4[idx + step], a2 = x4[idx + 2 * step], a3 = x4[idx + 3 * step];
            f32x4 b0 = a0, b1 = a0, b2 = a0, b3 = a0;
            if (HAS_Y) { b0 = y4[idx]; b1 = y4[idx + step]; b2 = y4[idx + 2 * step]; b3 = y4[idx + 3 * step]; }
            accumulate<MODE>(a0, b0, mu, is, ga, be, act, v);
            accumulate<MODE>(a1, b1, mu, is, ga, be, act, v);
            accumulate<MODE>(a2, b2, mu, is, ga, be, act, v);
            accumulate<MODE>(a3, b3, mu, is, ga, be, act, v);
        }
        for (; r < r_end; r += q.rpi, idx += step) {
            f32x4 a = x4[idx];
            f32x4 b = a;
            if (HAS_Y) b = y4[idx];
            accumulate<MODE>(a, b, mu, is, ga, be, act, v);
        }
    }
    block_fold<NQ>(q, ri, active, v);
    if (active && ri == 0) {
        const long o = (((long)g * q.P + p) * q.C4 + c4) * 4;
#pragma unroll
        for (int e = 0; e < 4; ++e) part1[o + e] = v[e];
        if (NQ == 8) {
#pragma unroll
            for (int e = 0; e < 4; ++e) part2[o + e] = v[4 + e];
        }
    }
}

__device__ __forceinline__ void chunk_sums(int G, int C, int P, const double* __restrict__ part1,
                                           const double* __restrict__ part2, int& idx, bool& lead, double& s1,
                                           double& s2) {
    __shared__ double sm1[NT], sm2[NT];
    const int cl = threadIdx.x & 15, pl = threadIdx.x >> 4;
    idx = blockIdx.x * 16 + cl;
    const bool ok = idx < G * C;
    double a = 0.0, b = 0.0;
    if (ok) {
        const int g = idx / C, c = idx % C;
        const long base = (long)g * P * C + c, step = 16L * C;
        int p = pl;
        for (; p + 48 < P; p += 64) {
            const long o = base + (long)p * C;
            double a0 = part1[o], a1 = part1[o + step], a2 = part1[o + 2 * step], a3 = part1[o + 3 * step];
            double b0 = 0.0, b1 = 0.0, b2 = 0.0, b3 = 0.0;
            if (part2) { b0 = part2[o]; b1 = part2[o + step]; b2 = part2[o + 2 * step]; b3 = part2[o + 3 * step]; }
            a += (a0 + a1) + (a2 + a3);
            b += (b0 + b1) + (b2 + b3);
        }
        for (; p < P; p += 16) {
            const long o = base + (long)p * C;
            a += part1[o];
            if (part2) b += part2[o];
        }
    }
    sm1[threadIdx.x] = a;
    sm2[threadIdx.x] = b;
    __syncthreads();
    lead = ok && pl == 0;
    if (lead) {
        for (int k = 1; k < 16; ++k) {
            a += sm1[k * 16 + cl];
            b += sm2[k * 16 + cl];
        }
    }
    s1 = a;
    s2 = b;
}

__global__ __launch_bounds__(NT) void stats_finalize(int G, int R, int C, int P, const double* __restrict__ part1,
                                                     const double* __restrict__ part2, float eps,
                                                     float* __restrict__ mean, float* __restrict__ invstd,
                                                     float* __restrict__ var_out, float momentum,
                                                     float* __restrict__ running_mean, float* __restrict__ running_var) {
    int idx; bool lead; double s1, s2;
    chunk_sums(G, C, P, part1, part2, idx, lead, s1, s2);
    if (!lead) return;
    const double n = (double)R;
    const double mu = s1 / n;
    double var = s2 / n - mu * mu;
    if (var < 0.0) var = 0.0;
    mean[idx] = (float)mu;
    invstd[idx] = (float)(1.0 / sqrt(var + (double)eps));
    if (var_out) var_out[idx] = (float)var;
    if (running_mean && G == 1) {
        const int c = idx;
        running_mean[c] = (1.f - momentum) * running_mean[c] + momentum * (float)mu;
        const double unb = (R > 1) ? var * n / (n - 1.0) : var;
        running_var[c] = (1.f - momentum) * running_var[c] + momentum * (float)unb;
    }
}

__global__ __launch_bounds__(NT) void normbwd_finalize(int G, int C, int P, const double* __restrict__ part1,
                                                       const double* __restrict__ part2, float* __restrict__ s1o,
                                                       float* __restrict__ s2o, float* __restrict__ dgamma,
                                                       float* __restrict__ dbeta) {
    int idx; bool lead; double s1, s2;
    chunk_sums(G, C, P, part1, part2, idx, lead, s1, s2);
    if (!lead) return;
    s1o[idx] = (float)s1;
    s2o[idx] = (float)s2;
    if (G == 1) {
        if (dbeta) dbeta[idx] = (float)s1;
        if (dgamma) dgamma[idx] = (float)s2;
    }
}

__global__ __launch_bounds__(NT) void partial_sum_finalize(int G, int C, int P, const double* __restrict__ part1,
                                                           float scale, float* __restrict__ out) {
    int idx; bool lead; double s1, s2;
    chunk_sums(G, C, P, part1, nullptr, idx, lead, s1, s2);
    if (lead) out[idx] = (float)(s1 * (double)scale);
}

__global__ void syncbn_combine(const float* __restrict__ st, int world, int C, double n_total, float eps,
                               float momentum, float* __restrict__ running_mean, float* __restrict__ running_var,
                               float* __restrict__ mean, float* __restrict__ invstd) {
    int c = blockIdx.x * blockDim.x + threadIdx.x;
    if (c >= C) return;
    double m = 0.0;
    for (int r = 0; r < world; ++r) m += (double)st[((long)r * 2) * C + c];
    m /= (double)world;
    double var = 0.0;
    for (int r = 0; r < world; ++r) {
        double d = (double)st[((long)r * 2) * C + c] - m;
        var += (double)st[((long)r * 2 + 1) * C + c] + d * d;
    }
    var /= (double)world;
    mean[c] = (float)m;
    invstd[c] = (float)(1.0 / sqrt(var + (double)eps));
    if (running_mean) {
        running_mean[c] = (1.f - momentum) * running_mean[c] + momentum * (float)m;
        const double unb = (n_total > 1.0) ? var * n_total / (n_total - 1.0) : var;
        running_var[c] = (1.f - momentum) * running_var[c] + momentum * (float)unb;
    }
}

__global__ __launch_bounds__(NT) void norm_apply_fwd(long total4, int R, int C4, const float* __restrict__ x,
                                                     const float* __restrict__ mean, const float* __restrict__ invstd,
                                                     const float* __restrict__ gamma, const float* __restrict__ beta,
                                                     int act, float* __restrict__ y) {
    const f32x4* x4 = reinterpret_cast<const f32x4*>(x);
    f32x4* y4 = reinterpret_cast<f32x4*>(y);
    for (long e = (long)blockIdx.x * NT + threadIdx.x; e < total4; e += (long)gridDim.x * NT) {
        long row = e / C4;
        int c4 = (int)(e - row * C4);
        long g = row / R;
        f32x4 a = x4[e];
        f32x4 mu = reinterpret_cast<const f32x4*>(mean)[g * C4 + c4];
        f32x4 is = reinterpret_cast<const f32x4*>(invstd)[g * C4 + c4];
        f32x4 ga = reinterpret_cast<const f32x4*>(gamma)[c4];
        f32x4 be = reinterpret_cast<const f32x4*>(beta)[c4];
        f32x4 o;
#pragma unroll
        for (int k = 0; k < 4; ++k) {
            float z = ga[k] * ((a[k] - mu[k]) * is[k]) + be[k];
            o[k] = ud_act(z, act);
        }
        y4[e] = o;
    }
}

__global__ __launch_bounds__(NT) void norm_apply_bwd(long total4, int R, int C4, const float* __restrict__ x,
                                                     const float* __restrict__ dy, const float* __restrict__ mean,
                                                     const float* __restrict__ invstd, const float* __restrict__ gamma,
                                                     const float* __restrict__ beta, const float* __restrict__ s1,
                                                     const float* __restrict__ s2, float invR, int act,
                                                     float* __restrict__ dx) {
    const f32x4* x4 = reinterpret_cast<const f32x4*>(x);
    const f32x4* dy4 = reinterpret_cast<const f32x4*>(dy);
    f32x4* dx4 = reinterpret_cast<f32x4*>(dx);
    for (long e = (long)blockIdx.x * NT + threadIdx.x; e < total4; e += (long)gridDim.x * NT) {
        long row = e / C4;
        int c4 = (int)(e - row * C4);
        long g = row / R;
        f32x4 a = x4[e], d = dy4[e];
        f32x4 mu = reinterpret_cast<const f32x4*>(mean)[g * C4 + c4];
        f32x4 is = reinterpret_cast<const f32x4*>(invstd)[g * C4 + c4];
        f32x4 ga = reinterpret_cast<const f32x4*>(gamma)[c4];
        f32x4 be = reinterpret_cast<const f32x4*>(beta)[c4];
        f32x4 t1 = reinterpret_cast<const f32x4*>(s1)[g * C4 + c4];
        f32x4 t2 = reinterpret_cast<const f32x4*>(s2)[g * C4 + c4];
        f32x4 o;
#pragma unroll
        for (int k = 0; k < 4; ++k) {
            float xh = (a[k] - mu[k]) * is[k];
            float dz = d[k];
            if (act) dz *= ud_act_grad(ga[k] * xh + be[k], act);
            o[k] = ga[k] * is[k] * (dz - t1[k] * invR - xh * t2[k] * invR);
        }
        dx4[e] = o;
    }
}

int ew_blocks(long total4) {
    long b = (total4 + NT - 1) / NT;
    if (b > 4096) b = 4096;
    if (b < 1) b = 1;
    return (int)b;
}

inline dim3 fin_grid(int G, int C) { return dim3((unsigned)ud_cdiv((long)G * C, 16)); }

}

extern "C" {

int ud_reduce_ws_doubles(int G, int R, int C) {
    if (G < 1 || R < 1 || C < 4 || C % 4) return UD_EINVAL;
    RedGeom q = make_geom(G, R, C);
    const long n = 2L * G * q.P * C;
    return n > 0x7fffffffL ? UD_EINVAL : (int)n;
}

int ud_norm_stats(const float* x, int G, int R, int C, float eps, double* ws, float* mean, float* invstd,
                  float* var_out, float momentum, float* running_mean, float* running_var, ud_stream_t stream) {
    if (C % 4 || G < 1 || R < 1 || !ws) return UD_EINVAL;
    hipStream_t s = (hipStream_t)stream;
    RedGeom q = make_geom(G, R, C);
    double* part1 = ws;
    double* part2 = ws + (long)G * q.P * C;
    hipLaunchKernelGGL(colreduce_partial<RED_STATS>, red_grid(q), dim3(NT), 0, s, q, x, nullptr, nullptr, nullptr,
                       nullptr, nullptr, 0, part1, part2);
    UD_LAUNCH_CHECK();
    hipLaunchKernelGGL(stats_finalize, fin_grid(G, C), dim3(NT), 0, s, G, R, C, q.P, part1, part2, eps, mean, invstd,
                       var_out, momentum, running_mean, running_var);
    UD_LAUNCH_CHECK();
    return 0;
}

int ud_syncbn_combine(const float* gathered, int world, int C, long rows_per_rank, float eps, float momentum,
                      float* running_mean, float* running_var, float* mean, float* invstd, ud_stream_t stream) {
    if (world < 1 || C < 1 || rows_per_rank < 1) return UD_EINVAL;
    hipLaunchKernelGGL(syncbn_combine, dim3(ud_cdiv(C, 256)), dim3(256), 0, (hipStream_t)stream, gathered, world, C,
                       (double)rows_per_rank * world, eps, momentum, running_mean, running_var, mean, invstd);
    UD_LAUNCH_CHECK();
    return 0;
}

int ud_norm_apply_fwd(const float* x, int G, int R, int C, const float* mean, const float* invstd, const float* gamma,
                      const float* beta, int act, float* y, ud_stream_t stream) {
    if (C % 4) return UD_EINVAL;
    long total4 = (long)G * R * (C / 4);
    hipLaunchKernelGGL(norm_apply_fwd, dim3(ew_blocks(total4)), dim3(NT), 0, (hipStream_t)stream, total4, R, C / 4, x,
                       mean, invstd, gamma, beta, act, y);
    UD_LAUNCH_CHECK();
    return 0;
}

int ud_norm_bwd(const float* x, const float* dy, int G, int R, int C, const float* mean, const float* invstd,
                const float* gamma, const float* beta, int act, double* ws, float* s1, float* s2, float* dgamma,
                float* dbeta, float* dx, ud_stream_t stream) {
    if (C % 4 || G < 1 || R < 1 || !ws || !s1 || !s2) return UD_EINVAL;
    hipStream_t s = (hipStream_t)stream;
    RedGeom q = make_geom(G, R, C);
    double* part1 = ws;
    double* part2 = ws + (long)G * q.P * C;
    hipLaunchKernelGGL(colreduce_partial<RED_NORMBWD>, red_grid(q), dim3(NT), 0, s, q, x, dy, mean, invstd, gamma, beta,
                       act, part1, part2);
    UD_LAUNCH_CHECK();
    hipLaunchKernelGGL(normbwd_finalize, fin_grid(G, C), dim3(NT), 0, s, G, C, q.P, part1, part2, s1, s2, dgamma, dbeta);
    UD_LAUNCH_CHECK();
    if (G > 1 && (dgamma || dbeta)) {
        ud_wgrad_fold f{};
        f.part = s1; f.aux = s2; f.dgamma = dgamma; f.dbeta = dbeta;
        f.kind = UD_FOLD_GROUP; f.nparts = G; f.n = C;
        const int rc = ud_param_fold_multi(&f, 1, stream);
        if (rc) return rc;
    }
    if (dx) {
        long total4 = (long)G * R * (C / 4);
        hipLaunchKernelGGL(norm_apply_bwd, dim3(ew_blocks(total4)), dim3(NT), 0, s, total4, R, C / 4, x, dy, mean,
                           invstd, gamma, beta, s1, s2, 1.f / (float)R, act, dx);
        UD_LAUNCH_CHECK();
    }
    return 0;
}

int ud_norm_bwd_apply(const float* x, const float* dy, int G, int R, int C, const float* mean, const float* invstd,
                      const float* gamma, const float* beta, const float* s1, const float* s2, float inv_count,
                      int act, float* dx, ud_stream_t stream) {
    if (C % 4 || G < 1 || R < 1) return UD_EINVAL;
    long total4 = (long)G * R * (C / 4);
    hipLaunchKernelGGL(norm_apply_bwd, dim3(ew_blocks(total4)), dim3(NT), 0, (hipStream_t)stream, total4, R, C / 4, x,
                       dy, mean, invstd, gamma, beta, s1, s2, inv_count, act, dx);
    UD_LAUNCH_CHECK();
    return 0;
}

int ud_group_colsum(const float* x, int G, int R, int C, float scale, double* ws, float* out, ud_stream_t stream) {
    if (C % 4 || G < 1 || R < 1 || !ws) return UD_EINVAL;
    hipStream_t s = (hipStream_t)stream;
    RedGeom q = make_geom(G, R, C);
    hipLaunchKernelGGL(colreduce_partial<RED_SUM>, red_grid(q), dim3(NT), 0, s, q, x, nullptr, nullptr, nullptr,
                       nullptr, nullptr, 0, ws, nullptr);
    UD_LAUNCH_CHECK();
    hipLaunchKernelGGL(partial_sum_finalize, fin_grid(G, C), dim3(NT), 0, s, G, C, q.P, ws, scale, out);
    UD_LAUNCH_CHECK();
    return 0;
}

int ud_group_coldot(const float* a, const float* b, int G, int R, int C, float scale, double* ws, float* out,
                    ud_stream_t stream) {
    if (C % 4 || G < 1 || R < 1 || !ws) return UD_EINVAL;
    hipStream_t s = (hipStream_t)stream;
    RedGeom q = make_geom(G, R, C);
    hipLaunchKernelGGL(colreduce_partial<RED_DOT>, red_grid(q), dim3(NT), 0, s, q, a, b, nullptr, nullptr, nullptr,
                       nullptr, 0, ws, nullptr);
    UD_LAUNCH_CHECK();
    hipLaunchKernelGGL(partial_sum_finalize, fin_grid(G, C), dim3(NT), 0, s, G, C, q.P, ws, scale, out);
    UD_LAUNCH_CHECK();
    return 0;
}

}
```

unidefense_amd/csrc/param_fold.hip:

```cpp
#include "ud_common.h"
#include "bnref.h"

namespace {

static_assert(NT == 256, "16 elements x 16 lanes of partials per workgroup");
constexpr int FOLD_MAX = 44;
struct FoldArgs {
    ud_wgrad_fold it[FOLD_MAX];
    int block0[FOLD_MAX + 1];
    int n;
};

__device__ __forceinline__ long out_index(int i, int KK, int B) {
    if (KK <= 1) return i;
    const int a = i / (KK * B), r = i - a * (KK * B), tap = r / B, b = r - tap * B;
    return ((long)a * B + b) * KK + tap;
}

__device__ __forceinline__ void fold_dw(const ud_wgrad_fold& f, int blk, double* smem) {
    double(*sm)[16][4] = reinterpret_cast<double(*)[16][4]>(smem);
    const int KK = f.p0 * f.p0, C = f.p1, KKC = KK * C, nparts = f.nparts;
    const int lane = threadIdx.x & 15, sl = threadIdx.x >> 4;
    const int i = (blk * 16 + lane) * 4;
    double v[4] = {0.0, 0.0, 0.0, 0.0};
    if (i < KKC) {
        const f32x4* p4 = reinterpret_cast<const f32x4*>(f.part + i);
        const long step = (long)KKC / 4;
        for (int p = sl; p < nparts; p += 16) {
            const f32x4 w = p4[(long)p * step];
#pragma unroll
            for (int e = 0; e < 4; ++e) v[e] += (double)w[e];
        }
    }
#pragma unroll
    for (int e = 0; e < 4; ++e) sm[sl][lane][e] = v[e];
    __syncthreads();
    if (sl < 4 && i < KKC) {
        double t = 0.0;
#pragma unroll
        for (int k = 0; k < 16; ++k) t += sm[k][lane][sl];
        const int o = i + sl, tap = o / C, c = o % C;
        f.dst[(long)c * KK + tap] = (float)(t * (double)gate_factor(f.aux, f.p2));
    }
}

__device__ __forceinline__ void fold_f32_lanes(const float* src, long st, int nparts, bool live, float* dst, float* smem) {
    float(*red)[17] = reinterpret_cast<float(*)[17]>(smem);
    const int el = threadIdx.x & 15, grp = threadIdx.x >> 4;
    float s0 = 0.f, s1 = 0.f;
    if (live) {
        int p = grp;
        for (; p + 16 < nparts; p += 32) {
            s0 += src[p * st];
            s1 += src[(p + 16) * st];
        }
        if (p < nparts) s0 += src[p * st];
    }
    red[grp][el] = s0 + s1;
    __syncthreads();
    if (grp == 0 && live) {
        float t = red[0][el];
#pragma unroll
        for (int j = 1; j < 16; ++j) t += red[j][el];
        *dst = t;
    }
}

__device__ __forceinline__ void fold_f32(const ud_wgrad_fold& f, int blk, double* smem) {
    const int i = blk * 16 + (threadIdx.x & 15);
    const bool live = i < f.n;
    fold_f32_lanes(f.part + i, f.n, f.nparts, live, live ? f.dst + out_index(i, f.p0, f.p1) : nullptr, reinterpret_cast<float*>(smem));
    const int c = blk * NT + threadIdx.x;
    if (c < f.p2) {
        if (f.dbeta) f.dbeta[c] = (float)f.s1l[c];
        if (f.dgamma) f.dgamma[c] = (float)f.s2l[c];
    }
}

__device__ __forceinline__ void fold_pj(const ud_wgrad_fold& f, int blk, double* smem) {
    const int CO = f.p0, CE = f.p1, CC = f.p2;
    const int i = blk * 16 + (threadIdx.x & 15);
    const bool live = i < f.n;
    const float* src = f.part;
    if (live) {
        const int co = i / CE, c = i - co * CE, chunk = c / CC, cc = c - chunk * CC;
        src += (long)chunk * f.nparts * (CO * CC) + co * CC + cc;
    }
    fold_f32_lanes(src, (long)CO * CC, f.nparts, live, f.dst + i, reinterpret_cast<float*>(smem));
}

__device__ __forceinline__ void fold_f64(const ud_wgrad_fold& f, int blk, double* sm) {
    const int el = threadIdx.x & 15, pl = threadIdx.x >> 4;
    const int i = blk * 16 + el, n = f.n;
    double acc = 0.0;
    if (i < n)
        for (int b = pl; b < f.nparts; b += 16) acc += (double)f.part[(long)b * n + i];
    sm[threadIdx.x] = acc;
    __syncthreads();
    if (pl == 0 && i < n) {
        for (int k = 1; k < 16; ++k) acc += sm[k * 16 + el];
        f.dst[out_index(i, f.p0, f.p1)] = (float)acc;
    }
}

__device__ __forceinline__ void fold_group(const ud_wgrad_fold& f, int blk) {
    const int c = blk * NT + threadIdx.x, C = f.n;
    if (c >= C) return;
    double a = 0.0, b = 0.0;
    for (int g = 0; g < f.nparts; ++g) {
        a += (double)f.part[(long)g * C + c];
        b += (double)f.aux[(long)g * C + c];
    }
    if (f.dbeta) f.dbeta[c] = (float)a;
    if (f.dgamma) f.dgamma[c] = (float)b;
}

__device__ __forceinline__ void fold_layout(const ud_wgrad_fold& f, int blk) {
    const int i = blk * NT + threadIdx.x;
    if (i < f.n) f.dst[out_index(i, f.p0, f.p1)] = f.part[i];
}

__global__ __launch_bounds__(NT) void param_fold_multi(const FoldArgs a) {
    __shared__ double sm[16 * 16 * 4];
    int j = 0;
    while (j + 1 < a.n && (int)blockIdx.x >= a.block0[j + 1]) ++j;
    const ud_wgrad_fold& f = a.it[j];
    const int blk = (int)blockIdx.x - a.block0[j];
    switch (f.kind) {
        case UD_FOLD_DW: fold_dw(f, blk, sm); break;
        case UD_FOLD_F32: fold_f32(f, blk, sm); break;
        case UD_FOLD_PJ: fold_pj(f, blk, sm); break;
        case UD_FOLD_F64: fold_f64(f, blk, sm); break;
        case UD_FOLD_GROUP: fold_group(f, blk); break;
        default: fold_layout(f, blk); break;
    }
}

int item_blocks(const ud_wgrad_fold& f) {
    if (!f.part || f.nparts < 1) return 0;
    const bool conv = f.kind == UD_FOLD_F32 || f.kind == UD_FOLD_F64 || f.kind == UD_FOLD_LAYOUT;
    if (conv && f.p0 > 1 && (f.p1 < 1 || f.n < 1 || f.n % (f.p0 * f.p1))) return 0;
    switch (f.kind) {
        case UD_FOLD_DW:
            if (!f.dst || (f.p0 != 3 && f.p0 != 5) || f.p1 < 4 || f.p1 % 4 || f.p2 < 0 || f.p2 > 2 || (f.p2 != 0 && !f.aux)) return 0;
            return ud_cdiv(f.p0 * f.p0 * f.p1, 64);
        case UD_FOLD_F32:
            if (!f.dst || f.n < 1 || f.p2 < 0 || f.p2 > 16L * f.n) return 0;
            if (f.p2 > 0 && ((f.dgamma && !f.s2l) || (f.dbeta && !f.s1l))) return 0;
            return ud_cdiv(f.n, 16);
        case UD_FOLD_PJ:
            if (!f.dst || f.p0 < 1 || f.p1 < 1 || f.p2 < 1 || f.p1 % f.p2 || f.n != f.p0 * f.p1) return 0;
            return ud_cdiv(f.n, 16);
        case UD_FOLD_F64:
            if (!f.dst || f.n < 1) return 0;
            return ud_cdiv(f.n, 16);
        case UD_FOLD_GROUP:
            if (!f.aux || f.n < 1 || (!f.dgamma && !f.dbeta)) return 0;
            return ud_cdiv(f.n, NT);
        case UD_FOLD_LAYOUT:
            if (!f.dst || f.n < 1 || f.dst == f.part) return 0;
            return ud_cdiv(f.n, NT);
        default: return 0;
    }
}

}

extern "C" {

int ud_param_fold_multi(const ud_wgrad_fold* items, int n, ud_stream_t stream) {
    if (!items || n < 1) return UD_EINVAL;
    for (int i = 0; i < n; ++i)
        if (item_blocks(items[i]) < 1) return UD_EINVAL;
    for (int i0 = 0; i0 < n; i0 += FOLD_MAX) {
        FoldArgs a;
        a.n = n - i0 < FOLD_MAX ? n - i0 : FOLD_MAX;
        int b = 0;
        for (int j = 0; j < a.n; ++j) {
            a.it[j] = items[i0 + j];
            a.block0[j] = b;
            b += item_blocks(a.it[j]);
        }
        a.block0[a.n] = b;
        hipLaunchKernelGGL(param_fold_multi, dim3((unsigned)b), dim3(NT), 0, (hipStream_t)stream, a);
        UD_LAUNCH_CHECK();
    }
    return 0;
}

}
```

unidefense_amd/kernels.py:

```python
import contextlib
import ctypes as C
import math
import os

import torch

from . import lib as _lib
from .config import cfg as CFG
from .devmem import Scratch, ZeroPool
from .lib import ConvGeom, GemmDesc, GemmP3Desc

_call = _lib.call
_const, _rows = _lib.const, _lib.const_rows

GEMM_PROFILE = None


def _stream():
    return C.c_void_p(torch.cuda.current_stream().cuda_stream)


def _p(t):
    if t is None:
        return None
# ... 2391 lines not shown
    if _fft_two_pass("rfft", S, h):
        _call("ud_rfft2_two_pass", _p(x), _p(Y), _p(_fft_ws(N, S, Cc, x)), N, S, Cc, scale, w_interior, None, None, None, 0,
              None, None, h, None, _stream())
        return Y
    _call("ud_rfft2", _p(x), _p(Y), N, S, Cc, scale, w_interior, h, _stream())
    return Y


def irfft2(Y, scale, w_interior=1.0):
    h = _act(Y)
    N, S, Wh, C2 = Y.shape
    assert Wh == S // 2 + 1 and C2 % 2 == 0
    if not fft_kernel_size(S):
        return _irfft2_generic(Y, scale, w_interior)
    x = empty((N, S, S, C2 // 2), Y, Y.dtype)
    if _fft_two_pass("irfft", S, h):
        _call("ud_irfft2_two_pass", _p(Y), _p(x), _p(_fft_ws(N, S, C2 // 2, Y)), N, S, C2 // 2, scale, w_interior, None, None,
              None, None, None, h, _stream())
        return x
    _call("ud_irfft2", _p(Y), _p(x), N, S, C2 // 2, scale, w_interior, h, _stream())
    return x


def fc_fwd(x, W, b, act_in=0):
    _chk(x, W, b)
    N, I = x.shape
    O = W.shape[0]
    y = empty((N, O), x)
    _call("ud_fc_fwd", _p(x), _p(W), _p(b), _p(y), N, I, O, act_in, _stream())
    return y


def fc_bwd(dy, W, x, act_in=0, need_dx=True, need_db=True, need_dw=True):
    _chk(dy, W, x)
    N, I = x.shape
    O = W.shape[0]
    dx = empty((N, I), x) if need_dx else None
    dW = empty((O, I), x) if need_dw else None
    db = empty((O,), x) if (need_db and need_dw) else None
    _call("ud_fc_bwd", _p(dy), _p(W), _p(x), _p(dx), _p(dW), _p(db), N, I, O, act_in, _stream())
    return dx, dW, db


def se_scale_fwd(x, s):
    _chk(x, s)
    N, H, W, Cc = x.shape
    y = torch.empty_like(x)
    _call("ud_se_scale_fwd", _p(x), _p(s), _p(y), N, H * W, Cc, _stream())
    return y


def se_scale_bwd(dy, s, dpool):
    _chk(dy, s, dpool)
    N, H, W, Cc = dy.shape
    dx = torch.empty_like(dy)
    _call("ud_se_scale_bwd", _p(dy), _p(s), _p(dpool), _p(dx), N, H * W, Cc, _stream())
    return dx


def sigmoid_grad_mul_(s, v):
    _chk(s, v)
    _call("ud_sigmoid_grad_mul", _p(s), _p(v), v.numel(), _stream())
    return v


def sfmix_fwd(spat, freq, alpha, pool):
    h = _act(spat, freq)
    _chk(alpha)
    N, Ho, Wo, Cc = spat.shape
    y = torch.empty_like(spat)
    _call("ud_sfmix_fwd", _p(spat), _p(freq), _p(alpha), _p(y), N, Ho, Wo, Cc, int(pool), h, _stream())
    return y


def sfmix_bwd(spat, freq, alpha, dy, pool):
    h = _act(spat, freq, dy)
    _chk(alpha)
    N, Ho, Wo, Cc = spat.shape
    nb = _call("ud_sfmix_blocks", N, Ho, Wo, Cc)
    part = torch.empty((nb,), dtype=torch.float64, device=spat.device)
    dspat = torch.empty_like(spat)
    dfreq = torch.empty_like(freq)
    dalpha = empty((), spat)
    _call("ud_sfmix_bwd", _p(spat), _p(freq), _p(alpha), _p(dy), _p(dspat), _p(dfreq), _p(part), _p(dalpha), N, Ho,
          Wo, Cc, int(pool), h, _stream())
    return dspat, dfreq, dalpha


def gate_mix_fwd(p, q, alpha):
    _chk(p, q, alpha)
    y = torch.empty_like(p)
    _call("ud_gate_mix_fwd", _p(p), _p(q), _p(alpha), _p(y), p.numel(), _stream())
    return y


def gate_mix_bwd(p, q, alpha, dy):
    _chk(p, q, alpha, dy)
    nb = _call("ud_gate_mix_blocks", p.numel())
    part = torch.empty((nb,), dtype=torch.float64, device=p.device)
    dp = torch.empty_like(p)
    dq = torch.empty_like(p)
    dalpha = empty((), p)
    _call("ud_gate_mix_bwd", _p(p), _p(q), _p(alpha), _p(dy), _p(dp), _p(dq), _p(part), _p(dalpha), p.numel(),
          _stream())
    return dp, dq, dalpha


def residual(x, skip, keep=None, inv_keep=1.0):
    _chk(x, skip, keep)
    out = torch.empty_like(x)
    _call("ud_residual_fwd", _p(x), _p(skip), _p(keep), inv_keep, _p(out), x.numel(), x.numel() // x.shape[0],
          _stream())
    return out


def axpby(a, alpha, b=None, beta=1.0, out=None):
    h = _act(a, b, out)
    if out is None:
        out = torch.empty_like(a)
    _call("ud_axpby", _p(a), alpha, _p(b), beta, _p(out), a.numel(), h, _stream())
    return out


def multi_add(dsts, srcs):
    n = len(dsts)
    if n == 0:
        return
    for d, s_ in zip(dsts, srcs):
        if not (d.is_cuda and s_.is_cuda and d.dtype == s_.dtype == torch.float32 and d.is_contiguous() and s_.is_contiguous()
                and d.numel() == s_.numel() and d.device == s_.device):
            raise ValueError("multi_add: contiguous float32 device tensors of equal sizes only")
    PA, LA = C.c_void_p * n, C.c_long * n
    _call("ud_multi_add", PA(*[d.data_ptr() for d in dsts]), PA(*[s_.data_ptr() for s_ in srcs]),
          LA(*[d.numel() for d in dsts]), n, _stream())


def mask_scale(x, mask, scale):
    _chk(x, mask)
    out = torch.empty_like(x)
    _call("ud_mask_scale", _p(x), _p(mask), scale, _p(out), x.numel(), _stream())
    return out


def absdiff(a, b=None):
    _chk(a, b)
    out = torch.empty_like(a)
    _call("ud_absdiff", _p(a), _p(b), _p(out), a.numel(), _stream())
    return out


def pix_to_planes(x, tanh=False):
    _chk(x)
    N, H, W, Cc = x.shape
    out = empty((N, Cc, H, W), x)
    _call("ud_pix_to_planes", _p(x), _p(out), N, Cc, H * W, 1 if tanh else 0, _stream())
    return out


def planes_to_pix(x, tanh_out=None):
    _chk(x, tanh_out)
    N, Cc, H, W = x.shape
    out = empty((N, H, W, Cc), x)
    _call("ud_planes_to_pix", _p(x), _p(tanh_out), _p(out), N, Cc, H * W, 2 if tanh_out is not None else 0,
          _stream())
    return out


def bilinear_fwd(x, Ho, Wo):
    _chk(x)
    N, Cc, Hi, Wi = x.shape
    y = empty((N, Cc, Ho, Wo), x)
    _call("ud_bilinear_fwd", _p(x), _p(y), N * Cc, Hi, Wi, Ho, Wo, _stream())
    return y


def bilinear_bwd(dy, Hi, Wi):
    _chk(dy)
    N, Cc, Ho, Wo = dy.shape
    dx = empty((N, Cc, Hi, Wi), dy)
    _call("ud_bilinear_bwd", _p(dy), _p(dx), N * Cc, Hi, Wi, Ho, Wo, _stream())
    return dx


def l1_fwd(a, b, scale):
    _chk(a, b)
    N = a.shape[0]
    per = a.numel() // N
    P = _call("ud_l1_chunks", per)
    part = empty((N, P), a)
    out = empty((N,), a)
    _call("ud_l1_fwd", _p(a), _p(b), _p(part), _p(out), N, per, scale, _stream())
    return out


def l1_bwd(a, b, g, scale, out=None):
    _chk(a, b, g, out)
    N = a.shape[0]
    acc = out is not None
    if out is None:
        out = torch.empty_like(a)
    _call("ud_l1_bwd", _p(a), _p(b), _p(g), scale, 1 if acc else 0, _p(out), N, a.numel() // N, _stream())
    return out


def dynfilter_fwd(proj2, diff2, w2, x2):
    _chk(proj2, diff2, w2, x2)
    M, Cc = proj2.shape
    D = diff2.shape[1]
    Cx = x2.shape[1]
    pre = empty((M, 2 + D), x2)
    argmax = torch.empty((M,), dtype=torch.int32, device=x2.device)
    mask = empty((M,), x2)
    out = torch.empty_like(x2)
    _call("ud_dynfilter_fwd", _p(proj2), _p(diff2), _p(w2), _p(x2), _p(pre), C.c_void_p(argmax.data_ptr()), _p(mask),
          _p(out), M, Cc, D, Cx, _stream())
    return out, mask, pre, argmax


def dynfilter_bwd(dout2, dmask_ext, x2, mask, argmax, w2, Cproj):
    _chk(dout2, dmask_ext, x2, mask, w2)
    M, Cx = x2.shape
    dx = torch.empty_like(x2)
    dlogit = empty((M,), x2)
    dproj = empty((M, Cproj), x2)
    _call("ud_dynfilter_bwd", _p(dout2), _p(dmask_ext), _p(x2), _p(mask), C.c_void_p(argmax.data_ptr()), _p(w2),
          _p(dx), _p(dlogit), _p(dproj), M, Cproj, Cx, _stream())
    return dx, dlogit, dproj


_DFT_CACHE = {}


def _dft_mats(S, device, ortho=True):
    key = (S, str(device), ortho)
    if key in _DFT_CACHE:
        return _DFT_CACHE[key]
    Wh = S // 2 + 1
    Whp = -(-Wh // 4) * 4
    Sp = -(-S // 4) * 4
    s = 1.0 / math.sqrt(S) if ortho else 1.0
    k = torch.arange(S, dtype=torch.float64)
    ang = 2.0 * math.pi * torch.outer(k, k) / S
    cosm, sinm = torch.cos(ang) * s, torch.sin(ang) * s
    fw_cos = torch.zeros(Whp, Sp, dtype=torch.float64)
    fw_sin = torch.zeros(Whp, Sp, dtype=torch.float64)
    fw_cos[:Wh, :S] = cosm[:Wh]
    fw_sin[:Wh, :S] = -sinm[:Wh]
    fh = torch.zeros(2 * S, 2 * Sp, dtype=torch.float64)
    fh[:S, :S], fh[:S, Sp:Sp + S] = cosm, sinm
    fh[S:, :S], fh[S:, Sp:Sp + S] = -sinm, cosm
    mats = tuple(m.to(torch.float32).to(device).contiguous() for m in (fw_cos, fw_sin, fh))
    _DFT_CACHE[key] = mats
    return mats


_FFT_PLANES_WS = Scratch(torch.float32)
_FFT_PLANES_SIZES = (128, 256, 320)


def _fft_planes_ws(ref, P, S):
    return _FFT_PLANES_WS.get(ref, _call("ud_rfft2_planes_ws_floats", P, S))


def dft_rfft2_planes(d, ortho=True):
    _chk(d)
    P, S, _ = d.shape
    if S in _FFT_PLANES_SIZES:
        Y = empty((P, 2 * S, -(-(S // 2 + 1) // 4) * 4), d)
        _call("ud_rfft2_planes", _p(d), _p(Y), _p(_fft_planes_ws(d, P, S)), P, S, (1.0 / S) if ortho else 1.0, _stream())
        return Y
    Sp = -(-S // 4) * 4
    if Sp != S:
        dp = torch.zeros((P, Sp, Sp), device=d.device)
        dp[:, :S, :S] = d
        d = dp
    return _dft_planes_fwd(d, S, ortho)


def _dft_planes_fwd(dp, S, ortho):
    P, Sp, _ = dp.shape
    fw_cos, fw_sin, fh = _dft_mats(S, dp.device, ortho)
    Whp = fw_cos.shape[0]
    d2 = dp.view(P * Sp, Sp)
    t_re = gemm_nt(d2, fw_cos)
    t_im = gemm_nt(d2, fw_sin)
    Y = empty((P, 2 * S, Whp), dp)
    _gemm(fh, t_re, Y, 2 * S, Whp, Sp, 2 * Sp, Whp, Whp, 0, 1, 0, batch=P, strideA=0, strideB=Sp * Whp,
          strideC=2 * S * Whp)
    _gemm(fh, t_im, Y, 2 * S, Whp, Sp, 2 * Sp, Whp, Whp, 0, 1, 1, batch=P, strideA=0, strideB=Sp * Whp,
          strideC=2 * S * Whp, a_off=Sp)
    return Y


def dft_rfft2_planes_adjoint(dY, S, ortho=True):
    _chk(dY)
    P = dY.shape[0]
    if S in _FFT_PLANES_SIZES:
        dd = empty((P, S, S), dY)
        _call("ud_rfft2_planes_adjoint", _p(dY), _p(dd), _p(_fft_planes_ws(dY, P, S)), P, S, (1.0 / S) if ortho else 1.0,
              _stream())
        return dd
    dd = _dft_planes_adj(dY, S, ortho)
    return dd if dd.shape[-1] == S else dd[:, :S, :S].contiguous()


def _dft_planes_adj(dY, S, ortho):
    P = dY.shape[0]
    fw_cos, fw_sin, fh = _dft_mats(S, dY.device, ortho)
    Whp, Sp = fw_cos.shape
    dt_re = empty((P * Sp, Whp), dY)
# ... 632 lines not shown
        dots, inv_hw, sacc = fold
        assert dots.numel() >= 5 * N * Cc and sacc.numel() >= 2 * Cc
        _call("ud_se_bwd_b_bn", _pd(ds1_acc), _p(s1), _p(Wr), _pd(pool), float(pool_scale), _p(dpool), _p(dWr), _p(dbr), _p(s2),
              _pd(dots), float(inv_hw), _pd(sacc), _pd(sacc, Cc), N, Cc, Cs, _stream())
        return dpool, dWe, dbe, dWr, dbr
    _call("ud_se_bwd_b", _pd(ds1_acc), _p(s1), _p(Wr), _pd(pool), float(pool_scale), _p(dpool), _p(dWr), _p(dbr), N, Cc,
          Cs, _stream())
    return dpool, dWe, dbe, dWr, dbr


def se_scale_bwd_bn(dc, x, bn, s, dpool, inv_hw, G, R, sacc):
    h = _act(dc, x)
    _chk(s, dpool)
    Cc = x.shape[-1]
    dz = torch.empty_like(x)
    _call("ud_se_scale_bwd_bn", _p(dc), _p(x), C.byref(bn.ref()), _p(s), _p(dpool), float(inv_hw), _p(dz), _pd(sacc),
          _pd(sacc, Cc), _fused_ws(x, G, R, Cc, False), G, R, Cc, h, _stream())
    return dz


def coldot_bn_eval(dy, x, bn, G, R, out):
    h = _act(dy, x)
    Cc = x.shape[-1]
    ws = _ws64(x, _call("ud_coldot_bn_eval_ws_doubles", G, R, Cc))
    _call("ud_coldot_bn_eval", _p(dy), _p(x), C.byref(bn.ref()), G, R, Cc, _pd(out), ws, h, _stream())


def se_scale_bwd_bn_eval(dc, x, bn, s, dpool, inv_hw, G, R):
    h = _act(dc, x)
    _chk(s, dpool)
    Cc = x.shape[-1]
    dd = torch.empty_like(x)
    _call("ud_se_scale_bwd_bn_eval", _p(dc), _p(x), C.byref(bn.ref()), _p(s), _p(dpool), float(inv_hw), _p(dd), G, R, Cc, h,
          _stream())
    return dd


def bn_eval_bwd(dy, x, bn, G, R):
    h = _act(dy, x)
    Cc = dy.shape[-1]
    dx = torch.empty_like(dy)
    _call("ud_bn_eval_bwd", _p(dy), _p(x), C.byref(bn.ref()), _p(dx), G, R, Cc, h, _stream())
    return dx


def sfmix_pool_bwd(dy):
    h = _act(dy)
    N, Ho, Wo, Cc = dy.shape
    df = empty((N, 2 * Ho, 2 * Wo, Cc), dy, dy.dtype)
    _call("ud_sfmix_pool_bwd", _p(dy), _p(df), N, Ho, Wo, Cc, h, _stream())
    return df


def dwconv_bwd_data_bn(dy, gate_alpha, gate_mode, wt, add, x, bn, K, stride, pad_t, pad_l, sacc):
    h = _act(dy, add, x)
    _chk(wt)
    N, H, W, Cc = x.shape
    _, Ho, Wo, _ = dy.shape
    dz = torch.empty_like(x)
    ws = _ws64(x, _call("ud_dwconv_bwd_data_bn_ws_doubles", N, H, W, Cc, stride))
    _call("ud_dwconv_bwd_data_bn", _p(dy), _p(gate_alpha), int(gate_mode), _p(wt), _p(add), _p(x), C.byref(bn.ref()),
          _p(dz), _pd(sacc), _pd(sacc, Cc), ws, N, H, W, Cc, Ho, Wo, K, stride, pad_t, pad_l, h, _stream())
    return dz


def dwconv_bwd_data_ex(dy, gate_alpha, gate_mode, wt, add, K, stride, pad_t, pad_l, H, W):
    h = _act(dy, add)
    _chk(wt)
    N, Ho, Wo, Cc = dy.shape
    dx = empty((N, H, W, Cc), dy, dy.dtype)
    _call("ud_dwconv_bwd_data_ex", _p(dy), _p(gate_alpha), int(gate_mode), _p(wt), _p(add), _p(dx), N, H, W, Cc, Ho, Wo,
          K, stride, pad_t, pad_l, h, _stream())
    return dx


def dwconv_bwd_weight_ex(x, dy, gate_alpha, gate_mode, K, stride, pad_t, pad_l):
    h = _act(x, dy)
    N, H, W, Cc = x.shape
    _, Ho, Wo, _ = dy.shape
    lanes = Cc // 2 if h else Cc
    chunks = max(1, min(N * Ho, -(-_DW_WGRAD_THREADS // lanes)))
    part = empty((chunks, K * K, Cc), x)
    dwt = empty((Cc, K * K), x)
    _call("ud_dwconv_bwd_weight_ex", _p(x), _p(dy), _p(gate_alpha), int(gate_mode), _p(dwt), _p(part), chunks, N, H, W,
          Cc, Ho, Wo, K, stride, pad_t, pad_l, h, _stream())
    return dwt


def rfft2_ex(x, scale, w_interior=1.0, bn=None, want_act=False, gate_alpha=None, gate_mode=0, update=False,
             gate_acc=None, want_absmax=False):
    h = _act(x)
    N, S, S2, Cc = x.shape
    assert S == S2
    Y = empty((N, S, S // 2 + 1, 2 * Cc), x, x.dtype)
    act = torch.empty_like(x) if (want_act and bn is not None) else None
    ggrad = empty((), x) if gate_acc is not None else None
    amax = amax_slots(x, want_absmax)
    Y._ud_absmax = amax
    tail = (C.byref(bn.ref(update)) if bn is not None else None, _p(act), _p(gate_alpha), int(gate_mode),
            _pd(gate_acc) if gate_acc is not None else None, _p(ggrad), h, _p(amax), _stream())
    if _fft_two_pass("rfft_ex", S, h):
        _call("ud_rfft2_two_pass", _p(x), _p(Y), _p(_fft_ws(N, S, Cc, x)), N, S, Cc, float(scale), float(w_interior), *tail)
    else:
        _call("ud_rfft2_ex", _p(x), _p(Y), N, S, Cc, float(scale), float(w_interior), *tail)
    return (Y, act, ggrad) if gate_acc is not None else (Y, act)


def rfft2_planes_ok(x, bn, stride_ok=True):
    if not (x.dtype == torch.float32 and CFG.spectral_p2 != "off"):
        return False
    N, S, _, Cc = x.shape
    return S in (8, 16, 32, 12, 24, 48) and (2 * Cc) % 32 == 0 and not _fft_two_pass("rfft_ex", S, 0)


def rfft2_dw_ok(S, k, stride, pad):
    return stride == 1 and S in (8, 16, 32) and k in (3, 5) and tuple(pad) == ((k - 1) // 2,) * 4


def rfft2_ex_planes(x, scale, w_interior=1.0, bn=None, want_act=False, gate_alpha=None, gate_mode=0, update=False,
                    gate_acc=None, energy=None, dw_wt=None, dw_k=0):
    _chk(x)
    N, S, S2, Cc = x.shape
    assert S == S2 and (bn is not None or energy is not None)
    R = N * S * (S // 2 + 1)
    pl = Planes(R, 2 * Cc, x, 2, False)
    act = torch.empty_like(x) if (want_act and bn is not None) else None
    ggrad = empty((), x) if gate_acc is not None else None
    pre = float(scale) * max(1.0, float(w_interior)) * S
    if energy is None:
        pre *= math.sqrt(float(bn.count))
    spat = torch.empty_like(x) if dw_k else None
    _call("ud_rfft2_ex_planes", _p(x), _p(pl.buf), pl.panel, pl.plane, _p(pl.inv), pre, _pd(energy) if energy is not None else None,
          N, S, Cc, float(scale), float(w_interior), C.byref(bn.ref(update)) if bn is not None else None, _p(act), _p(gate_alpha),
          int(gate_mode), _pd(gate_acc) if gate_acc is not None else None, _p(ggrad), _p(dw_wt), _p(spat), int(dw_k), _stream())
    out = (pl, act, ggrad) if gate_acc is not None else (pl, act)
    return out + (spat,) if dw_k else out


def irfft2_mix(Y, scale, spat, alpha, acc):
    h = _act(Y, spat)
    _chk(alpha)
    N, S, Wh, C2 = Y.shape
    Cc = C2 // 2
    assert spat.shape == (N, S, S, Cc)
    y = torch.empty_like(spat)
    fr = torch.empty_like(spat)
    s1, s2 = (_pd(acc), _pd(acc, Cc)) if acc is not None else (None, None)
    if _fft_two_pass("irfft_mix", S, h):
        _call("ud_irfft2_two_pass", _p(Y), _p(y), _p(_fft_ws(N, S, Cc, Y)), N, S, Cc, float(scale), 1.0, _p(spat), _p(alpha),
              _p(fr), s1, s2, h, _stream())
    else:
        _call("ud_irfft2_mix", _p(Y), _p(y), N, S, Cc, float(scale), 1.0, _p(spat), _p(alpha), _p(fr), s1, s2, h, _stream())
    return y, fr


def _bnp(bn, update=False):
    return C.byref(bn.ref(update)) if bn is not None else None


def dwtile_fwd(x, wt, K, pad_t, pad_l, Ho, Wo, bn=None, stats=None, update=False, stride=1):
    h = _act(x)
    _chk(wt)
    N, H, W, Cc = x.shape
    y = empty((N, Ho, Wo, Cc), x, x.dtype)
    ws = None
    if stats is not None:
        ws = _ws64(x, _call("ud_dwtile_ws_doubles", N, Ho, Wo, Cc))
    _call("ud_dwtile", _p(x), _bnp(bn, update), _p(wt), _p(y), N, H, W, Cc, Ho, Wo, K, pad_t, pad_l, 0, None, 0, None, None,
          None, 1 if stats is not None else 0, _pd(stats) if stats is not None else None,
          _pd(stats, Cc) if stats is not None else None, ws, int(stride), h, _stream())
    return y


def dwtile_bwd_data(dy, wt, K, pad_t, pad_l, H, W, gate_alpha=None, gate_mode=0, add=None, x=None, bn=None, sacc=None,
                    stride=1):
    h = _act(dy, add, x)
    _chk(wt)
    N, Ho, Wo, Cc = dy.shape
    out = empty((N, H, W, Cc), dy, dy.dtype)
    ws = None
    if bn is not None:
        ws = _ws64(dy, _call("ud_dwtile_ws_doubles", N, H, W, Cc))
    _call("ud_dwtile", _p(dy), None, _p(wt), _p(out), N, Ho, Wo, Cc, H, W, K, K - 1 - pad_t, K - 1 - pad_l, 1,
          _p(gate_alpha), int(gate_mode), _p(add), _p(x) if bn is not None else None, _bnp(bn), 2,
          _pd(sacc) if bn is not None else None, _pd(sacc, Cc) if bn is not None else None, ws, int(stride), h, _stream())
    return out


def dwtile_dgrad_eval(dy, wt, K, pad_t, pad_l, x, bn, gate_alpha=None, gate_mode=0, add=None, stride=1):
    h = _act(dy, add, x)
    _chk(wt)
    N, H, W, Cc = x.shape
    _, Ho, Wo, _ = dy.shape
    dx = torch.empty_like(x)
    _call("ud_dwtile_dgrad_eval", _p(dy), _p(wt), _p(gate_alpha), int(gate_mode), _p(add), _p(x), C.byref(bn.ref()), _p(dx),
          N, H, W, Cc, Ho, Wo, K, pad_t, pad_l, int(stride), h, _stream())
    return dx


_WGRAD_FOLDS = None
_WGRAD_PART_WS = Scratch(torch.float32)
_FOLDS_IMMEDIATE = False
FOLD_KINDS = _rows("UD_FOLD_")


@contextlib.contextmanager
def immediate_folds():
    global _FOLDS_IMMEDIATE
    prev, _FOLDS_IMMEDIATE = _FOLDS_IMMEDIATE, True
    try:
        yield
    finally:
        _FOLDS_IMMEDIATE = prev


def begin_wgrad_folds():
    global _WGRAD_FOLDS
    if _WGRAD_FOLDS:
        flush_wgrad_folds()
    _WGRAD_FOLDS = None if _FOLDS_IMMEDIATE else []


def flush_wgrad_folds(end=False):
    global _WGRAD_FOLDS
    items = _WGRAD_FOLDS
    if items:
        from .lib import WgradFold
        arr = (WgradFold * len(items))()
        for a, (fields, _keep, _dsts) in zip(arr, items):
            for k, v in fields.items():
                setattr(a, k, v.data_ptr() if isinstance(v, torch.Tensor) else v)
        _call("ud_param_fold_multi", arr, len(items), _stream())
        for _fields, _keep, dsts in items:
            for t in dsts:
                t._ud_deferred = False
    _WGRAD_FOLDS = None if (end or items is None) else []


def folds_deferred():
    return _WGRAD_FOLDS is not None


def _wgrad_part(like, need, ws=None):
    if _WGRAD_FOLDS is not None:
        return torch.empty(need, dtype=torch.float32, device=like.device), True
    return (_WGRAD_PART_WS if ws is None else ws).get(like, need), False


def _defer_fold(kind, dsts, keep=(), **fields):
    for t in dsts:
        t._ud_deferred = True
    fields["kind"] = FOLD_KINDS[kind]
    _WGRAD_FOLDS.append((fields, tuple(keep) + tuple(v for v in fields.values() if isinstance(v, torch.Tensor)), tuple(dsts)))


def _defer_wgrad_fold(part, nparts, K_, Cc, gate_alpha, gate_mode, dwt):
    _defer_fold("dw", (dwt,), part=part, dst=dwt, aux=gate_alpha if gate_mode else None, nparts=int(nparts), p0=int(K_), p1=int(Cc),
                p2=int(gate_mode))


def dwtile_bwd_weight(x, dy, K, pad_t, pad_l, bn=None, gate_alpha=None, gate_mode=0, stride=1):
    h = _act(x, dy)
    N, H, W, Cc = x.shape
    _, Ho, Wo, _ = dy.shape
    rows = _call("ud_dwtile_wgrad_part_rows", N, Ho, Wo)
    part, defer = _wgrad_part(x, rows * K * K * Cc)
    dwt = empty((Cc, K * K), x)
    nparts = _call("ud_dwtile_wgrad", _p(x), _bnp(bn), _p(dy), _p(gate_alpha), int(gate_mode), None if defer else _p(dwt), _p(part),
                   rows, N, H, W, Cc, Ho, Wo, K, pad_t, pad_l, int(stride), h, _stream())
    if defer:
        _defer_wgrad_fold(part, nparts, K, Cc, gate_alpha, gate_mode, dwt)
    return dwt


def dwtile_bwd(dy, x, wt, K, pad_t, pad_l, bn=None, gate_alpha=None, gate_mode=0, add=None, sacc=None):
    h = _act(dy, x, add)
    _chk(wt)
    N, H, W, Cc = x.shape
    assert dy.shape == x.shape
    rows = _call("ud_dwtile_wgrad_part_rows", N, H, W)
    part, defer = _wgrad_part(x, rows * K * K * Cc)
    dz = empty((N, H, W, Cc), dy, dy.dtype)
# ... 70 lines not shown
```

unidefense_amd/loss/pass_tail.py:

```python
import torch
import torch.nn as nn

from .triplet_loss import AsymmetricalWeightedTripletLoss

_KEYS = ("total", "cls", "triplet", "real_rec", "fake_rec", "real_freq", "fake_freq", "freq_mask", "spat_mask")


class _PassTail(torch.autograd.Function):
    @staticmethod
    def forward(ctx, n_real, n_fake, weights, tgt, nfeat, cls_out, fm, sm, spatial, freq, *feats):
        from .. import kernels as K

        def c(t):
            return None if t is None else t.detach().contiguous()
        vals, grads = K.loss_tail(c(cls_out), tgt.contiguous(), n_real, n_fake, [c(f) for f in feats], c(fm), c(sm), c(spatial),
                                  c(freq), weights)
        ctx.grads = grads
        ctx.shapes = [None if t is None else t.shape for t in (cls_out, fm, sm, spatial, freq)]
        outs = vals.unbind(0)
        ctx.mark_non_differentiable(*outs[1:])
        return outs

    @staticmethod
    def backward(ctx, g, *_):
        grads = ctx.grads
        flat = grads["_flat"] * g
        base = grads["_flat"].data_ptr()

        def view(k, shape=None):
            t = grads.get(k)
            if t is None:
                return None
            off = (t.data_ptr() - base) // 4
            return flat[off:off + t.numel()].view(t.shape if shape is None else shape)
        sh = ctx.shapes
        nfeat = sum(1 for k in grads if k.startswith("feat"))
        return (None, None, None, None, None, view("cls", sh[0]), view("fm", sh[1]), view("sm", sh[2]), view("spatial", sh[3]),
                view("freq", sh[4])) + tuple(view(f"feat{i}") for i in range(nfeat))


def pass_tail(out_dict, tgt, n_real, n_fake, criteria, weights, masks=True):
    cls_out = out_dict["cls_out"]
    ld = out_dict.get("loss_dict", {})
    feats = ld.get("triplet")
    fm, sm = (ld.get("freq_mask"), ld.get("spat_mask")) if masks else (None, None)
    spatial, freq = ld.get("spatial"), ld.get("freq")
    ce, trip = criteria.get("softmax"), criteria.get("triplet")
    N = cls_out.shape[0]
    ok = (cls_out.is_cuda and cls_out.dtype == torch.float32 and cls_out.dim() == 2 and 2 <= cls_out.shape[-1] <= 64
          and type(ce) is nn.CrossEntropyLoss and ce.weight is None and ce.ignore_index == -100 and ce.reduction == "mean"
          and ce.label_smoothing == 0.0 and tgt.dtype == torch.int64 and tgt.shape == (N,)
          and n_real is not None and n_fake is not None and 0 < n_real < N and n_real + n_fake <= N
          and (feats is None or (type(trip) is AsymmetricalWeightedTripletLoss and len(feats) <= 3
                                 and all(f.dim() == 2 and f.shape[0] == N and f.dtype == torch.float32 for f in feats)))
          and all(t is None or (t.dtype == torch.float32 and t.is_cuda) for t in (fm, sm, spatial, freq))
          and all(t is None or t.shape == (N,) for t in (spatial, freq)))
    if not ok:
        return None
    feats = list(feats) if feats is not None else []
    w = (weights["cls"], weights["mask"], weights["mask"], weights["triplet"], weights["rec"], weights["freq"])
    outs = _PassTail.apply(int(n_real), int(n_fake), w, tgt, len(feats), cls_out, fm, sm, spatial, freq, *feats)
    return dict(zip(_KEYS, outs))
```

unidefense_amd/model/unidefense.py:

```python
from typing import List, Optional

import torch
import torch.nn as nn

from .. import kernels as K
from ..config import cfg
from .. import mbconv as MB
from .. import tape as T
from .arch import DELIMITER_DICT, build_arch


class _SFConvParams(nn.Conv2d):

    def __init__(self, channels, k):
        super().__init__(channels, channels, k, groups=channels, bias=False)
        self.freq_conv = nn.Conv2d(channels * 2, channels * 2, kernel_size=1, bias=False)
        self.sf_coef = nn.Parameter(torch.tensor(-10.0))


class _MBConvParams(nn.Module):

    def __init__(self, spec, eps, momentum):
        super().__init__()
        self.spec = spec
# ... 5 lines not shown
        else:
            self._depthwise_conv = nn.Conv2d(spec.cexp, spec.cexp, spec.k, groups=spec.cexp, bias=False)
        self._bn1 = nn.BatchNorm2d(spec.cexp, momentum=momentum, eps=eps)
        self._se_reduce = nn.Conv2d(spec.cexp, spec.cse, 1)
        self._se_expand = nn.Conv2d(spec.cse, spec.cexp, 1)
        self._project_conv = nn.Conv2d(spec.cexp, spec.cout, 1, bias=False)
        self._bn2 = nn.BatchNorm2d(spec.cout, momentum=momentum, eps=eps)


class _Backbone(nn.Module):

    def __init__(self, arch):
        super().__init__()
        eps, mom = arch["bn_eps"], arch["bn_momentum"]
        self._conv_stem = nn.Conv2d(3, arch["stem"]["cout"], 3, stride=2, bias=False)
        self._bn0 = nn.BatchNorm2d(arch["stem"]["cout"], momentum=mom, eps=eps)
        self._blocks = nn.ModuleList([_MBConvParams(s, eps, mom) for s in arch["blocks"]])
        self._conv_head = nn.Conv2d(arch["head"]["cin"], arch["head"]["cout"], 1, bias=False)
        self._bn1 = nn.BatchNorm2d(arch["head"]["cout"], momentum=mom, eps=eps)


class Classifier(nn.Module):

    def __init__(self, depth=512, num_classes=2):
        super().__init__()
        self.fc = nn.Linear(depth, num_classes)
        self.fc.weight.data.normal_(0, 0.01)
        self.fc.bias.data.fill_(0.0)


class _FilterParams(nn.Module):

    def __init__(self, cin, k, d_in, affine, bias):
        super().__init__()
        self.layer1 = nn.Sequential(nn.Conv2d(cin, cin, k, 1, k // 2, bias=bias), nn.BatchNorm2d(cin, affine=affine),
                                    nn.Identity())
        self.layer2 = nn.Sequential(nn.Conv2d(d_in, 1, 1, bias=bias), nn.Identity())


def _decoder(cin, cout, affine, bias, last):
    mods = [nn.Conv2d(cin, cout, 3, 1, 1, bias=bias), nn.InstanceNorm2d(cout, affine=affine), nn.Identity(),
            nn.ConvTranspose2d(cout, cout, 3, 2, 1, output_padding=1, bias=bias),
            nn.InstanceNorm2d(cout, affine=affine), nn.Identity(),
            nn.Conv2d(cout, cout, 3, 1, 1, bias=bias), nn.InstanceNorm2d(cout, affine=affine), nn.Identity()]
    if last:
        mods += [nn.Conv2d(cout, 3, 3, 1, 1, bias=bias), nn.Identity()]
    return nn.Sequential(*mods)


_OUT_KEYS = ("cls_out", "rec", "factorization", "triplet0", "triplet1", "triplet2", "freq_mask", "spat_mask",
             "spatial", "freq")


def _fused_mbconv():
    return cfg.fused_mbconv


def _half_storage(model):
    return bool(getattr(model, "half_storage", cfg.half_storage))


_MULTI_ADD_MIN = 8


def _accumulate_in_place(model, params, grads):
    if not getattr(model, "_ud_inplace_accumulate", False) or torch.is_grad_enabled():
        return grads
    idx = [i for i, (p, g) in enumerate(zip(params, grads))
           if g is not None and p.grad is not None and p.grad.dtype == torch.float32 and g.dtype == torch.float32
           and p.grad.is_contiguous() and p.grad.shape == g.shape and p.grad.device == g.device and not p.grad.requires_grad
           and not p._backward_hooks and not getattr(p, "_post_accumulate_grad_hooks", None)]
    if len(idx) < _MULTI_ADD_MIN:
        return grads
    K.multi_add([params[i].grad for i in idx], [grads[i].contiguous() for i in idx])
    grads = list(grads)
    for i in idx:
        grads[i] = None
    return grads


class _NetFunction(torch.autograd.Function):
    @staticmethod
    def forward(ctx, model, x, noise_x, rng, *params):
        K.begin_forward(model)
        tape = T.Tape()
        if ctx.needs_input_grad[1] and noise_x is None:
            tape.input = x
        tape.wgrad_on = model.training or any(ctx.needs_input_grad[4:])
        debug = getattr(model, "_debug_watch", False)
        if debug:
            tape.kinks = {}
        try:
            outs = model._run(x, tape, rng, noise_x)
            tape.weight_snapshot = K.weight_batch_snapshot()
        finally:
            K.end_forward()
        if debug:
            tape.watch = {id(t): k for k, t in outs["_feats"].items()}
            model._debug_tape = tape
            model._debug_feats = outs["_feats"]
            names = {id(p): n[: -len(".weight")] for n, p in model.named_parameters() if n.endswith(".weight")}
            model._debug_kinks = {names.get(k, k): (y > 0) for k, y in tape.kinks.items()}
        ctx.tape = tape
        ctx.outs = outs
        ctx.params = params
        ctx.x_tracked = tape.input is not None
        ctx.model = model
        ctx.keys = model._out_keys
        return tuple(outs[k] for k in ctx.keys)

    @staticmethod
    def backward(ctx, *gouts):
        tape, outs, model = ctx.tape, ctx.outs, ctx.model
        K.reset_zero_pool()
        reducer = getattr(model, "_grad_reducer", None) if tape.wgrad_on else None
        scale = getattr(model, "_grad_prescale", 1.0) if reducer is not None else 1.0
        uses = getattr(model, "_param_uses", None)
        if reducer is not None:
            reducer.begin()
            if uses is not None:
                tape.param_uses, tape.param_ready = uses, reducer.ready
        for k, g in zip(ctx.keys, gouts):
            if g is not None:
                g = g.contiguous().to(torch.float32)
                tape.add_grad(outs[k], g if scale == 1.0 else g * scale)
        tape.backward()
        grads = [tape.param_grads.get(p) if p.requires_grad else None for p in ctx.params]
        if reducer is not None:
            if uses is None:
                model._param_uses = dict(tape.param_seen)
            elif uses != tape.param_seen:
                raise RuntimeError("data parallel: the set of parameter-gradient contributions changed between "
                                   "backward passes; streamed buckets would hold partial gradients")
            for p, g in zip(reversed(ctx.params), reversed(grads)):
                if g is not None and id(p) not in reducer.done:
                    reducer.ready(id(p), g)
            red = reducer.finish()
            grads = [None if g is None else red[id(p)] for p, g in zip(ctx.params, grads)]
        grads = _accumulate_in_place(model, ctx.params, grads)
        dx = tape.input_grad if ctx.x_tracked else None
        if dx is not None and scale != 1.0:
            dx = K.axpby(dx, 1.0 / scale)
        tape.input = tape.input_grad = None
        ctx.tape = ctx.outs = ctx.model = None
        return (None, dx, None, None) + tuple(grads)


class RunnerMethods:

    def inference_runner(self, batch, size, precision="fp32"):
        from ..infer import inference_runner
        return inference_runner(self, batch, size, precision)

    def input_grad_runner(self, batch, size, objective="cross_entropy", precision="fp32", grad_scale=None):
        from ..attack import input_grad_runner
        return input_grad_runner(self, batch, size, objective, precision, grad_scale)

    def attack_runner(self, batch, size, **kwargs):
        from ..attack import attack_runner
        return attack_runner(self, batch, size, **kwargs)

    def apgd_runner(self, batch, size, **kwargs):
        from ..attack import apgd_runner
        return apgd_runner(self, batch, size, **kwargs)

    def fmn_runner(self, batch, size, **kwargs):
# ... 370 lines not shown
```

unidefense_amd/tape.py:

```python
import math
from typing import Optional

import torch

from . import kernels as K
from .config import cfg


class Tape:

    def __init__(self):
        self.nodes = []
        self.grads = {}
        self.param_grads = {}
        self._keep = []
        self.watch = None
        self.captured = {}
        self.kinks = None
        self.gate_cond = {}
        self.param_ready = None
        self.param_uses = None
        self.param_seen = {}
        self._deferred = set()
        self.weight_snapshot = None
# ... 609 lines not shown
    y = K.planes_to_pix(x)
    if _needs(tape):
        def bwd():
            dy = tape.pop_grad(y)
            if dy is not None:
                tape.add_grad(x, K.pix_to_planes(dy.contiguous()))
        tape.record(bwd)
    return y


def absdiff(tape, a, b):
    y = K.absdiff(a, b)
    if _needs(tape):
        def bwd():
            dy = tape.pop_grad(y)
            if dy is not None:
                tape.add_grad(b, K.absdiff_bwd(a, b, dy.contiguous()))
        tape.record(bwd)
    return y


def attention_diffs(tape, pred_planes, x, h, w, norm):
    pred = K.planes_to_pix(K.bilinear_fwd(pred_planes, h, w))
    sf, _ = _fft_scales(h, norm)
    if not _tracks(tape, x):
        xs = K.planes_to_pix(K.bilinear_fwd(x, h, w))
        return K.absdiff(K.rfft2(pred, sf), K.rfft2(xs, sf)), K.absdiff(pred, xs), False
    xs = planes_to_pix(tape, bilinear(tape, x, h, w))
    freq_diff = absdiff(tape, K.rfft2(pred, sf), rfft2_cat(tape, xs, norm))
    return freq_diff, absdiff(tape, pred, xs), True


def rec_losses(tape, rec, x, norm):
    N, Cc, S, _ = rec.shape
    assert norm == "ortho", "frequency reconstruction loss implemented for freq_norm='ortho'"
    cnt_s = Cc * S * S
    Wh = S // 2 + 1
    cnt_f = Cc * S * Wh
    spatial = K.l1_fwd(rec, x, 1.0 / cnt_s)
    d = K.axpby(rec, 1.0, x, -1.0)
    Y = K.dft_rfft2_planes(d.view(N * Cc, S, S))
    freq = K.l1_fwd(Y.view(N, -1), None, 1.0 / cnt_f)
    if _needs(tape):
        def bwd():
            gs = tape.pop_grad(spatial)
            gf = tape.pop_grad(freq)
            grec = tape.pop_grad(rec)
            if gs is None and gf is None and grec is None:
                return
            total = None
            if gf is not None:
                dY = K.l1_bwd(Y.view(N, -1), None, gf, 1.0 / cnt_f).view(Y.shape)
                total = K.dft_rfft2_planes_adjoint(dY, S).view(rec.shape)
            if gs is not None:
                total = K.l1_bwd(rec, x, gs, 1.0 / cnt_s, out=total)
            if total is not None and _tracks(tape, x):
                tape.add_grad(x, K.axpby(total, -1.0))
            if grec is not None:
                total = grec if total is None else K.axpby(total, 1.0, grec, 1.0)
            tape.grads[id(rec)] = total
            tape._keep.append(rec)
        tape.record(bwd)
    return spatial, freq


def dynamic_filter(tape, x, proj, diff, w2, b2=None, diff_grad=False):
    Cx, Cp, D = x.shape[-1], proj.shape[-1], diff.shape[-1]
    x2, p2, d2 = x.view(-1, Cx), proj.view(-1, Cp), diff.view(-1, D)
    w2f = w2.view(-1)
    if b2 is not None:
        d2 = torch.cat([d2, torch.ones_like(d2[:, :1])], 1)
        w2f = torch.cat([w2f.detach(), b2.detach().view(-1)])
    out2, mask, pre, argmax = K.dynfilter_fwd(p2, d2, w2f, x2)
    out = out2.view(x.shape)
    mask4 = mask.view(*x.shape[:-1], 1)
    if _needs(tape):
        def bwd():
            dout = tape.pop_grad(out)
            dmask = tape.pop_grad(mask4)
            if dout is None and dmask is None:
                return
            if dout is None:
                dout = torch.zeros_like(out)
            dx, dlogit, dproj = K.dynfilter_bwd(dout.view(-1, Cx), None if dmask is None else dmask.view(-1),
                                                x2, mask, argmax, w2f, Cp)
            tape.add_grad(x, dx.view(x.shape))
            tape.add_grad(proj, dproj.view(proj.shape))
            if diff_grad:
                tape.add_grad(diff, K.outer(dlogit, w2f[2:2 + D]).view(diff.shape))
            if not _wgrad(tape):
                return
            g = K.gemm_tn(dlogit.view(-1, 1), pre)
            if b2 is None:
                tape.add_param_grad(w2, g.view(w2.shape))
            else:
                tape.add_param_grad(w2, g[:, :-1].reshape(w2.shape))
                tape.add_param_grad(b2, g[:, -1].reshape(b2.shape))
        tape.record(bwd)
    return out, mask4


def conv_dense_any(tape, x, w, stride, pad, need_dx=True, x_planes=None):
    N, Hin, Win, Ci = x.shape
    Co, _, KH, KW = w.shape
    Hout = (Hin + 2 * pad - KH) // stride + 1
    Wout = (Win + 2 * pad - KW) // stride + 1
    g = K.conv_geom(N, Hin, Win, Ci, Hout, Wout, KH, KW, stride, pad, pad, 0)
    wmat = K.weight_layout(w, 0)
    stem_dx = _tracks(tape, x_planes)
    if K.conv_im2col_ok(g, Co, x):
        assert not stem_dx
        return _conv_im2col(tape, x, w, wmat, g, need_dx)
    y = K.conv_gather_nt(x, wmat, g)
    if _needs(tape):
        wd = K.weight_layout(w, 2) if need_dx else None

        def bwd():
            dy = tape.pop_grad(y)
            if dy is None:
                return
            if need_dx:
                gd = K.conv_geom(N, Hout, Wout, Co, Hin, Win, KH, KW, stride, pad, pad, 1)
                tape.add_grad(x, K.conv_gather_nt(dy, wd, gd))
            elif stem_dx:
                _stem_dgrad(tape, dy, w, g, x_planes)
            if _wgrad(tape):
                tape.add_param_grad(w, K.conv_wgrad_param(dy.view(-1, Co), x, g))
        tape.record(bwd)
    return y


def sfconv_dense(tape, x, w, w_freq, alpha, stride, norm, bias=None):
    spat = bias_add(tape, conv_dense_any(tape, x, w, stride, 1), bias)
    xf = rfft2_cat(tape, x, norm)
    yf = conv1x1(tape, xf, w_freq)
    fr = irfft2_split(tape, yf, norm)
    return sfmix(tape, spat, fr, alpha)


def add_relu(tape, a, b, site=None):
    y = K.add_act(a, b, 2)
    if tape is not None and tape.kinks is not None and site is not None:
        tape.kinks[site] = y
    if _needs(tape):
        def bwd():
            dy = tape.pop_grad(y)
            if dy is None:
                return
            g = K.relu_bwd(dy, y)
            tape.add_grad(a, g)
            tape.add_grad(b, g)
        tape.record(bwd)
    return y


def avgpool(tape, x, k):
    if k == 1:
        return x
    y = K.avgpool_fwd(x, k)
    if _needs(tape):
        def bwd():
            dy = tape.pop_grad(y)
            if dy is None:
                return
            tape.add_grad(x, K.avgpool_bwd(dy, k))
        tape.record(bwd)
    return y


def maxpool3s2(tape, x, return_arg=False):
    H, W = x.shape[1], x.shape[2]
    y, arg = K.maxpool3s2_fwd(x)
    if _needs(tape):
        def bwd():
            dy = tape.pop_grad(y)
            if dy is None:
                return
            tape.add_grad(x, K.maxpool3s2_bwd(dy, arg, H, W))
        tape.record(bwd)
    return (y, arg) if return_arg else y
# ... 62 lines not shown
```

Baseline: 1496.

## Fuse small-reduction finalizes into fold batching and single-pass norm reductions

Depthwise weight-grad and gate-grad finalize kernels are moved into the shared deferred parameter-fold launcher, so they batch with other folds instead of each taking its own launch. The dynamic-filter backward now computes its weight-gradient partials inside the same kernel, replacing a separate tiny GEMM. Column reductions with a single partial chunk write final stats directly and skip the finalize kernel. Autograd grad materialization is disabled to avoid zero-filled gradient tensors. The aim is fewer small launches in backward, at the cost of extra code paths and mode switches.

```diff
diff --git a/include/unidefense_hip.h b/include/unidefense_hip.h
--- a/include/unidefense_hip.h
+++ b/include/unidefense_hip.h
@@ -82,6 +82,8 @@
 int ud_weight_layouts_multi(const ud_layout_item* items_dev, int n, int blocks_total, ud_stream_t stream);
 
 int ud_reduce_ws_doubles(int G, int R, int C);
+int ud_norm_finish_single(int on);
+int ud_reduce_chunks(int G, int R, int C);
 int ud_norm_stats(const float* x, int G, int R, int C, float eps, double* ws, float* mean, float* invstd,
                   float* var_out, float momentum, float* running_mean, float* running_var, ud_stream_t stream);
 int ud_syncbn_combine(const float* gathered, int world, int C, long rows_per_rank, float eps, float momentum,
@@ -161,6 +163,10 @@
 int ud_dynfilter_bwd(const float* dout, const float* dmask_ext, const float* x, const float* mask,
                      const int* argmax, const float* w2, float* dx, float* dlogit, float* dproj, int M,
                      int C, int Cx, ud_stream_t stream);
+int ud_dynfilter_bwd_blocks(int M);
+int ud_dynfilter_bwd_w(const float* dout, const float* dmask_ext, const float* x, const float* mask, const int* argmax,
+                       const float* w2, const float* pre, float* dx, float* dlogit, float* dproj, float* wpart, float* dw2,
+                       int M, int C, int Cx, int J, ud_stream_t stream);
 
 int ud_avgpool_fwd(const float* x, float* y, int N, int Ho, int Wo, int C, int k, ud_stream_t stream);
 int ud_avgpool_bwd(const float* dy, float* dx, int N, int Ho, int Wo, int C, int k, ud_stream_t stream);
@@ -608,6 +614,8 @@
 #define UD_FOLD_F64 3
 #define UD_FOLD_GROUP 4
 #define UD_FOLD_LAYOUT 5
+#define UD_FOLD_DW4 6
+#define UD_FOLD_GATE 7
 typedef struct {
     const float* part;
     float* dst;
diff --git a/unidefense_amd/csrc/fused.hip b/unidefense_amd/csrc/fused.hip
--- a/unidefense_amd/csrc/fused.hip
+++ b/unidefense_amd/csrc/fused.hip
@@ -1065,42 +1065,6 @@
     for (int i = 0; i < K * K; ++i) *reinterpret_cast<VF*>(out + (long)i * C) = acc[i];
 }
 
-__global__ __launch_bounds__(NT) void dw_bwd_weight_finalize_ex(int nparts, int KK, int C, const float* __restrict__ part,
-                                                                const float* __restrict__ gate_alpha, int gate_mode,
-                                                                float* __restrict__ dw) {
-    const int KKC = KK * C;
-    __shared__ double sm[16][16][4];
-    const int lane = threadIdx.x & 15, sl = threadIdx.x >> 4;
-    const int i = (blockIdx.x * 16 + lane) * 4;
-    double a[4] = {0.0, 0.0, 0.0, 0.0};
-    if (i < KKC) {
-        const f32x4* p4 = reinterpret_cast<const f32x4*>(part + i);
-        const long step = (long)KKC / 4;
-        int p = sl;
-        for (; p + 48 < nparts; p += 64) {
-            const f32x4 v0 = p4[(long)p * step], v1 = p4[(long)(p + 16) * step];
-            const f32x4 v2 = p4[(long)(p + 32) * step], v3 = p4[(long)(p + 48) * step];
-#pragma unroll
-            for (int e = 0; e < 4; ++e) a[e] += ((double)v0[e] + (double)v1[e]) + ((double)v2[e] + (double)v3[e]);
-        }
-        for (; p < nparts; p += 16) {
-            const f32x4 v = p4[(long)p * step];
-#pragma unroll
-            for (int e = 0; e < 4; ++e) a[e] += (double)v[e];
-        }
-    }
-#pragma unroll
-    for (int e = 0; e < 4; ++e) sm[sl][lane][e] = a[e];
-    __syncthreads();
-    if (sl < 4 && i < KKC) {
-        double t = 0.0;
-#pragma unroll
-        for (int k = 0; k < 16; ++k) t += sm[k][lane][sl];
-        const int o = i + sl, tap = o / C, c = o % C;
-        dw[(long)c * KK + tap] = (float)(t * (double)gate_factor(gate_alpha, gate_mode));
-    }
-}
-
 inline bool dw_geom_ok(const DwGeom& q, int K) {
     return q.N > 0 && q.H > 0 && q.W > 0 && q.C4 > 0 && q.Ho > 0 && q.Wo > 0 && (q.stride == 1 || q.stride == 2) &&
            (K == 3 || K == 5);
@@ -1593,7 +1557,7 @@
 int ud_dwconv_bwd_weight_ex(const void* x, const void* dy, const float* gate_alpha, int gate_mode, float* dwt,
                             float* part, int chunks, int N, int H, int W, int C, int Ho, int Wo, int K, int stride,
                             int pad_t, int pad_l, int f16, ud_stream_t stream) {
-    if (C % 4 || chunks < 1 || !x || !dy || !dwt || !part) return UD_EINVAL;
+    if (C % 4 || chunks < 1 || !x || !dy || !part) return UD_EINVAL;
     DwGeom q{N, H, W, C / 4, Ho, Wo, stride, pad_t, pad_l};
     if (!dw_geom_ok(q, K)) return UD_EINVAL;
     hipStream_t s = (hipStream_t)stream;
@@ -1612,11 +1576,11 @@
     else UD_DW_WG(5, 2);
 #undef UD_DW_WG
     UD_LAUNCH_CHECK();
-    const int KKC = K * K * C;
-    hipLaunchKernelGGL(dw_bwd_weight_finalize_ex, dim3(ud_cdiv(KKC, 64)), dim3(NT), 0, s, chunks, K * K, C, part,
-                       gate_alpha, gate_mode, dwt);
-    UD_LAUNCH_CHECK();
-    return 0;
-}
-
-}
+    if (!dwt) return chunks;
+    ud_wgrad_fold f{};
+    f.part = part; f.dst = dwt; f.aux = gate_alpha;
+    f.kind = UD_FOLD_DW4; f.nparts = chunks; f.p0 = K; f.p1 = C; f.p2 = gate_alpha ? gate_mode : 0;
+    return ud_param_fold_multi(&f, 1, stream);
+}
+
+}
diff --git a/unidefense_amd/csrc/misc.hip b/unidefense_amd/csrc/misc.hip
--- a/unidefense_amd/csrc/misc.hip
+++ b/unidefense_amd/csrc/misc.hip
@@ -226,20 +226,12 @@
     }
 }
 
-__global__ __launch_bounds__(NT) void gate_grad_finalize(int n, const double* __restrict__ part,
-                                                         const float* __restrict__ alpha, float* __restrict__ out) {
-    double acc = 0.0;
-    for (int i = threadIdx.x; i < n; i += NT) acc += part[i];
-    __shared__ double sm[NT / 64];
-    acc = ud_wave_sum_d(acc);
-    if ((threadIdx.x & 63) == 0) sm[threadIdx.x >> 6] = acc;
-    __syncthreads();
-    if (threadIdx.x == 0) {
-        double tot = 0.0;
-        for (int i = 0; i < NT / 64; ++i) tot += sm[i];
-        double a = 1.0 / (1.0 + exp(-(double)alpha[0]));
-        out[0] = (float)(tot * a * (1.0 - a));
-    }
+int gate_grad_fold(int n, const double* part, const float* alpha, float* out, hipStream_t s) {
+    if (!out) return n;
+    ud_wgrad_fold f{};
+    f.s1l = part; f.aux = alpha; f.dst = out;
+    f.kind = UD_FOLD_GATE; f.nparts = n;
+    return ud_param_fold_multi(&f, 1, (ud_stream_t)s);
 }
 
 
@@ -499,27 +491,40 @@
     for (int c = lane; c < Cx; c += 64) out[(long)m * Cx + c] = mk * x[(long)m * Cx + c];
 }
 
+template <bool WG>
 __global__ __launch_bounds__(NT) void dynfilter_bwd(int M, int C, int Cx, const float* __restrict__ dout,
                                                     const float* __restrict__ dmask_ext, const float* __restrict__ x,
                                                     const float* __restrict__ mask, const int* __restrict__ argmax,
                                                     const float* __restrict__ w2, float* __restrict__ dx,
-                                                    float* __restrict__ dlogit, float* __restrict__ dproj) {
+                                                    float* __restrict__ dlogit, float* __restrict__ dproj,
+                                                    const float* __restrict__ pre, int J, float* __restrict__ wpart) {
     const int m = (blockIdx.x * NT + threadIdx.x) >> 6, lane = threadIdx.x & 63;
-    if (m >= M) return;
-    const float mk = mask[m];
-    float acc = 0.f;
-    for (int c = lane; c < Cx; c += 64) {
-        float d = dout[(long)m * Cx + c];
-        acc += d * x[(long)m * Cx + c];
-        dx[(long)m * Cx + c] = mk * d;
-    }
-    acc = ud_wave_sum(acc);
-    const float dm = acc + (dmask_ext ? dmask_ext[m] : 0.f);
-    const float dl = dm * mk * (1.f - mk);
-    if (lane == 0) dlogit[m] = dl;
-    const float gm = dl * w2[0] / (float)C, gx = dl * w2[1];
-    const int am = argmax[m];
-    for (int c = lane; c < C; c += 64) dproj[(long)m * C + c] = gm + ((c == am) ? gx : 0.f);
+    double wprod = 0.0;
+    if (m < M) {
+        const float mk = mask[m];
+        float acc = 0.f;
+        for (int c = lane; c < Cx; c += 64) {
+            float d = dout[(long)m * Cx + c];
+            acc += d * x[(long)m * Cx + c];
+            dx[(long)m * Cx + c] = mk * d;
+        }
+        acc = ud_wave_sum(acc);
+        const float dm = acc + (dmask_ext ? dmask_ext[m] : 0.f);
+        const float dl = dm * mk * (1.f - mk);
+        if (lane == 0) dlogit[m] = dl;
+        const float gm = dl * w2[0] / (float)C, gx = dl * w2[1];
+        const int am = argmax[m];
+        for (int c = lane; c < C; c += 64) dproj[(long)m * C + c] = gm + ((c == am) ? gx : 0.f);
+        if (WG && lane < J) wprod = (double)dl * (double)pre[(long)m * J + lane];
+    }
+    if (WG) {
+        __shared__ double sm[NT];
+        sm[threadIdx.x] = wprod;
+        __syncthreads();
+        if (threadIdx.x < J)
+            wpart[(long)blockIdx.x * J + threadIdx.x] =
+                (float)(((sm[threadIdx.x] + sm[64 + threadIdx.x]) + sm[128 + threadIdx.x]) + sm[192 + threadIdx.x]);
+    }
 }
 
 struct DwWtEntry { const float* src; long C, KK, dst_off; };
@@ -646,9 +651,7 @@
                                                 (const T*)spat, (const T*)freq, alpha, (const T*)dy, (T*)dspat,
                                                 (T*)dfreq, part));
     UD_LAUNCH_CHECK();
-    hipLaunchKernelGGL(gate_grad_finalize, dim3(1), dim3(NT), 0, s, nb, part, alpha, dalpha);
-    UD_LAUNCH_CHECK();
-    return 0;
+    return gate_grad_fold(nb, part, alpha, dalpha, s);
 }
 
 int ud_sfmix_pool_bwd(const void* dy, void* dfreq, int N, int Ho, int Wo, int C, int f16, ud_stream_t stream) {
@@ -674,9 +677,7 @@
     int nb = ew_blocks(total, 1024);
     hipLaunchKernelGGL(gate_mix_bwd, dim3(nb), dim3(NT), 0, s, total, p, q, alpha, dy, dp, dq, part);
     UD_LAUNCH_CHECK();
-    hipLaunchKernelGGL(gate_grad_finalize, dim3(1), dim3(NT), 0, s, nb, part, alpha, dalpha);
-    UD_LAUNCH_CHECK();
-    return 0;
+    return gate_grad_fold(nb, part, alpha, dalpha, s);
 }
 
 int ud_residual_fwd(const float* x, const float* skip, const float* keep, float inv_keep, float* out, long total,
@@ -792,10 +793,27 @@
 int ud_dynfilter_bwd(const float* dout, const float* dmask_ext, const float* x, const float* mask, const int* argmax,
                      const float* w2, float* dx, float* dlogit, float* dproj, int M, int C, int Cx,
                      ud_stream_t stream) {
-    hipLaunchKernelGGL(dynfilter_bwd, dim3(ud_cdiv((long)M * 64, NT)), dim3(NT), 0, (hipStream_t)stream, M, C, Cx, dout,
-                       dmask_ext, x, mask, argmax, w2, dx, dlogit, dproj);
-    UD_LAUNCH_CHECK();
-    return 0;
+    hipLaunchKernelGGL(dynfilter_bwd<false>, dim3(ud_cdiv((long)M * 64, NT)), dim3(NT), 0, (hipStream_t)stream, M, C, Cx, dout,
+                       dmask_ext, x, mask, argmax, w2, dx, dlogit, dproj, nullptr, 0, nullptr);
+    UD_LAUNCH_CHECK();
+    return 0;
+}
+
+int ud_dynfilter_bwd_blocks(int M) { return M < 1 ? UD_EINVAL : (int)ud_cdiv((long)M * 64, NT); }
+
+int ud_dynfilter_bwd_w(const float* dout, const float* dmask_ext, const float* x, const float* mask, const int* argmax,
+                       const float* w2, const float* pre, float* dx, float* dlogit, float* dproj, float* wpart, float* dw2, int M,
+                       int C, int Cx, int J, ud_stream_t stream) {
+    if (M < 1 || J < 1 || J > 64 || !pre || !wpart) return UD_EINVAL;
+    const int blocks = (int)ud_cdiv((long)M * 64, NT);
+    hipLaunchKernelGGL(dynfilter_bwd<true>, dim3(blocks), dim3(NT), 0, (hipStream_t)stream, M, C, Cx, dout, dmask_ext, x, mask,
+                       argmax, w2, dx, dlogit, dproj, pre, J, wpart);
+    UD_LAUNCH_CHECK();
+    if (!dw2) return blocks;
+    ud_wgrad_fold f{};
+    f.part = wpart; f.dst = dw2;
+    f.kind = UD_FOLD_F64; f.nparts = blocks; f.n = J;
+    return ud_param_fold_multi(&f, 1, stream);
 }
 
 int ud_dw_weights_tapmajor(const void* table, int layers, long max_elems, float* dst, ud_stream_t stream) {
diff --git a/unidefense_amd/csrc/norm.hip b/unidefense_amd/csrc/norm.hip
--- a/unidefense_amd/csrc/norm.hip
+++ b/unidefense_amd/csrc/norm.hip
@@ -29,13 +29,50 @@
     }
 }
 
-template <int MODE>
+struct FinOut {
+    int R;
+    float eps, momentum, scale;
+    float *mean, *invstd, *var_out, *running_mean, *running_var;
+    float *s1, *s2, *dgamma, *dbeta;
+    float* out;
+};
+
+__device__ __forceinline__ void stats_outputs(int G, int R, int idx, double s1, double s2, float eps, float* __restrict__ mean,
+                                              float* __restrict__ invstd, float* __restrict__ var_out, float momentum,
+                                              float* __restrict__ running_mean, float* __restrict__ running_var) {
+    const double n = (double)R;
+    const double mu = s1 / n;
+    double var = s2 / n - mu * mu;
+    if (var < 0.0) var = 0.0;
+    mean[idx] = (float)mu;
+    invstd[idx] = (float)(1.0 / sqrt(var + (double)eps));
+    if (var_out) var_out[idx] = (float)var;
+    if (running_mean && G == 1) {
+        const int c = idx;
+        running_mean[c] = (1.f - momentum) * running_mean[c] + momentum * (float)mu;
+        const double unb = (R > 1) ? var * n / (n - 1.0) : var;
+        running_var[c] = (1.f - momentum) * running_var[c] + momentum * (float)unb;
+    }
+}
+
+__device__ __forceinline__ void normbwd_outputs(int G, int idx, double s1, double s2, float* __restrict__ s1o,
+                                                float* __restrict__ s2o, float* __restrict__ dgamma, float* __restrict__ dbeta) {
+    s1o[idx] = (float)s1;
+    s2o[idx] = (float)s2;
+    if (G == 1) {
+        if (dbeta) dbeta[idx] = (float)s1;
+        if (dgamma) dgamma[idx] = (float)s2;
+    }
+}
+
+template <int MODE, bool FIN>
 __global__ __launch_bounds__(NT) void colreduce_partial(RedGeom q, const float* __restrict__ x,
                                                         const float* __restrict__ y2,
                                                         const float* __restrict__ mean,
                                                         const float* __restrict__ invstd,
                                                         const float* __restrict__ gamma, const float* __restrict__ beta,
-                                                        int act, double* __restrict__ part1, double* __restrict__ part2) {
+                                                        int act, double* __restrict__ part1, double* __restrict__ part2,
+                                                        const FinOut fo) {
     constexpr bool HAS_Y = (MODE == RED_NORMBWD || MODE == RED_DOT);
     constexpr int NQ = (MODE == RED_STATS || MODE == RED_NORMBWD) ? 8 : 4;
     int ri, c4;
@@ -76,6 +113,22 @@
         }
     }
     block_fold<NQ>(q, ri, active, v);
+    if (FIN) {
+        if (active && ri == 0) {
+#pragma unroll
+            for (int e = 0; e < 4; ++e) {
+                const int idx = (g * q.C4 + c4) * 4 + e;
+                if (MODE == RED_STATS)
+                    stats_outputs(q.G, fo.R, idx, v[e], v[4 + e], fo.eps, fo.mean, fo.invstd, fo.var_out, fo.momentum, fo.running_mean,
+                                  fo.running_var);
+                else if (MODE == RED_NORMBWD)
+                    normbwd_outputs(q.G, idx, v[e], v[4 + e], fo.s1, fo.s2, fo.dgamma, fo.dbeta);
+                else
+                    fo.out[idx] = (float)(v[e] * (double)fo.scale);
+            }
+        }
+        return;
+    }
     if (active && ri == 0) {
         const long o = (((long)g * q.P + p) * q.C4 + c4) * 4;
 #pragma unroll
@@ -135,19 +188,7 @@
     int idx; bool lead; double s1, s2;
     chunk_sums(G, C, P, part1, part2, idx, lead, s1, s2);
     if (!lead) return;
-    const double n = (double)R;
-    const double mu = s1 / n;
-    double var = s2 / n - mu * mu;
-    if (var < 0.0) var = 0.0;
-    mean[idx] = (float)mu;
-    invstd[idx] = (float)(1.0 / sqrt(var + (double)eps));
-    if (var_out) var_out[idx] = (float)var;
-    if (running_mean && G == 1) {
-        const int c = idx;
-        running_mean[c] = (1.f - momentum) * running_mean[c] + momentum * (float)mu;
-        const double unb = (R > 1) ? var * n / (n - 1.0) : var;
-        running_var[c] = (1.f - momentum) * running_var[c] + momentum * (float)unb;
-    }
+    stats_outputs(G, R, idx, s1, s2, eps, mean, invstd, var_out, momentum, running_mean, running_var);
 }
 
 __global__ __launch_bounds__(NT) void normbwd_finalize(int G, int C, int P, const double* __restrict__ part1,
@@ -157,12 +198,7 @@
     int idx; bool lead; double s1, s2;
     chunk_sums(G, C, P, part1, part2, idx, lead, s1, s2);
     if (!lead) return;
-    s1o[idx] = (float)s1;
-    s2o[idx] = (float)s2;
-    if (G == 1) {
-        if (dbeta) dbeta[idx] = (float)s1;
-        if (dgamma) dgamma[idx] = (float)s2;
-    }
+    normbwd_outputs(G, idx, s1, s2, s1o, s2o, dgamma, dbeta);
 }
 
 __global__ __launch_bounds__(NT) void partial_sum_finalize(int G, int C, int P, const double* __restrict__ part1,
@@ -261,9 +297,23 @@
 
 inline dim3 fin_grid(int G, int C) { return dim3((unsigned)ud_cdiv((long)G * C, 16)); }
 
+bool g_finish_single = true;
+inline bool finishes(const RedGeom& q) { return q.P == 1 && g_finish_single; }
+
 }
 
 extern "C" {
+
+int ud_norm_finish_single(int on) {
+    const int prev = g_finish_single ? 1 : 0;
+    g_finish_single = on != 0;
+    return prev;
+}
+
+int ud_reduce_chunks(int G, int R, int C) {
+    if (G < 1 || R < 1 || C < 4 || C % 4) return UD_EINVAL;
+    return make_geom(G, R, C).P;
+}
 
 int ud_reduce_ws_doubles(int G, int R, int C) {
     if (G < 1 || R < 1 || C < 4 || C % 4) return UD_EINVAL;
@@ -279,8 +329,17 @@
     RedGeom q = make_geom(G, R, C);
     double* part1 = ws;
     double* part2 = ws + (long)G * q.P * C;
-    hipLaunchKernelGGL(colreduce_partial<RED_STATS>, red_grid(q), dim3(NT), 0, s, q, x, nullptr, nullptr, nullptr,
-                       nullptr, nullptr, 0, part1, part2);
+    if (finishes(q)) {
+        FinOut fo{};
+        fo.R = R; fo.eps = eps; fo.momentum = momentum;
+        fo.mean = mean; fo.invstd = invstd; fo.var_out = var_out; fo.running_mean = running_mean; fo.running_var = running_var;
+        hipLaunchKernelGGL((colreduce_partial<RED_STATS, true>), red_grid(q), dim3(NT), 0, s, q, x, nullptr, nullptr, nullptr,
+                           nullptr, nullptr, 0, nullptr, nullptr, fo);
+        UD_LAUNCH_CHECK();
+        return 0;
+    }
+    hipLaunchKernelGGL((colreduce_partial<RED_STATS, false>), red_grid(q), dim3(NT), 0, s, q, x, nullptr, nullptr, nullptr,
+                       nullptr, nullptr, 0, part1, part2, FinOut{});
     UD_LAUNCH_CHECK();
     hipLaunchKernelGGL(stats_finalize, fin_grid(G, C), dim3(NT), 0, s, G, R, C, q.P, part1, part2, eps, mean, invstd,
                        var_out, momentum, running_mean, running_var);
@@ -315,11 +374,19 @@
     RedGeom q = make_geom(G, R, C);
     double* part1 = ws;
     double* part2 = ws + (long)G * q.P * C;
-    hipLaunchKernelGGL(colreduce_partial<RED_NORMBWD>, red_grid(q), dim3(NT), 0, s, q, x, dy, mean, invstd, gamma, beta,
-                       act, part1, part2);
-    UD_LAUNCH_CHECK();
-    hipLaunchKernelGGL(normbwd_finalize, fin_grid(G, C), dim3(NT), 0, s, G, C, q.P, part1, part2, s1, s2, dgamma, dbeta);
-    UD_LAUNCH_CHECK();
+    if (finishes(q)) {
+        FinOut fo{};
+        fo.s1 = s1; fo.s2 = s2; fo.dgamma = dgamma; fo.dbeta = dbeta;
+        hipLaunchKernelGGL((colreduce_partial<RED_NORMBWD, true>), red_grid(q), dim3(NT), 0, s, q, x, dy, mean, invstd, gamma, beta,
+                           act, nullptr, nullptr, fo);
+        UD_LAUNCH_CHECK();
+    } else {
+        hipLaunchKernelGGL((colreduce_partial<RED_NORMBWD, false>), red_grid(q), dim3(NT), 0, s, q, x, dy, mean, invstd, gamma, beta,
+                           act, part1, part2, FinOut{});
+        UD_LAUNCH_CHECK();
+        hipLaunchKernelGGL(normbwd_finalize, fin_grid(G, C), dim3(NT), 0, s, G, C, q.P, part1, part2, s1, s2, dgamma, dbeta);
+        UD_LAUNCH_CHECK();
+    }
     if (G > 1 && (dgamma || dbeta)) {
         ud_wgrad_fold f{};
         f.part = s1; f.aux = s2; f.dgamma = dgamma; f.dbeta = dbeta;
@@ -351,8 +418,16 @@
     if (C % 4 || G < 1 || R < 1 || !ws) return UD_EINVAL;
     hipStream_t s = (hipStream_t)stream;
     RedGeom q = make_geom(G, R, C);
-    hipLaunchKernelGGL(colreduce_partial<RED_SUM>, red_grid(q), dim3(NT), 0, s, q, x, nullptr, nullptr, nullptr,
-                       nullptr, nullptr, 0, ws, nullptr);
+    if (finishes(q)) {
+        FinOut fo{};
+        fo.scale = scale; fo.out = out;
+        hipLaunchKernelGGL((colreduce_partial<RED_SUM, true>), red_grid(q), dim3(NT), 0, s, q, x, nullptr, nullptr, nullptr,
+                           nullptr, nullptr, 0, nullptr, nullptr, fo);
+        UD_LAUNCH_CHECK();
+        return 0;
+    }
+    hipLaunchKernelGGL((colreduce_partial<RED_SUM, false>), red_grid(q), dim3(NT), 0, s, q, x, nullptr, nullptr, nullptr,
+                           nullptr, nullptr, 0, ws, nullptr, FinOut{});
     UD_LAUNCH_CHECK();
     hipLaunchKernelGGL(partial_sum_finalize, fin_grid(G, C), dim3(NT), 0, s, G, C, q.P, ws, scale, out);
     UD_LAUNCH_CHECK();
@@ -364,8 +439,16 @@
     if (C % 4 || G < 1 || R < 1 || !ws) return UD_EINVAL;
     hipStream_t s = (hipStream_t)stream;
     RedGeom q = make_geom(G, R, C);
-    hipLaunchKernelGGL(colreduce_partial<RED_DOT>, red_grid(q), dim3(NT), 0, s, q, a, b, nullptr, nullptr, nullptr,
-                       nullptr, 0, ws, nullptr);
+    if (finishes(q)) {
+        FinOut fo{};
+        fo.scale = scale; fo.out = out;
+        hipLaunchKernelGGL((colreduce_partial<RED_DOT, true>), red_grid(q), dim3(NT), 0, s, q, a, b, nullptr, nullptr, nullptr,
+                           nullptr, 0, nullptr, nullptr, fo);
+        UD_LAUNCH_CHECK();
+        return 0;
+    }
+    hipLaunchKernelGGL((colreduce_partial<RED_DOT, false>), red_grid(q), dim3(NT), 0, s, q, a, b, nullptr, nullptr, nullptr,
+                           nullptr, 0, ws, nullptr, FinOut{});
     UD_LAUNCH_CHECK();
     hipLaunchKernelGGL(partial_sum_finalize, fin_grid(G, C), dim3(NT), 0, s, G, C, q.P, ws, scale, out);
     UD_LAUNCH_CHECK();
diff --git a/unidefense_amd/csrc/param_fold.hip b/unidefense_amd/csrc/param_fold.hip
--- a/unidefense_amd/csrc/param_fold.hip
+++ b/unidefense_amd/csrc/param_fold.hip
@@ -4,12 +4,13 @@
 namespace {
 
 static_assert(NT == 256, "16 elements x 16 lanes of partials per workgroup");
-constexpr int FOLD_MAX = 44;
+constexpr int FOLD_MAX = 45;
 struct FoldArgs {
     ud_wgrad_fold it[FOLD_MAX];
     int block0[FOLD_MAX + 1];
     int n;
 };
+static_assert(sizeof(FoldArgs) + 256 <= 4096, "the items travel in the kernel arguments");
 
 __device__ __forceinline__ long out_index(int i, int KK, int B) {
     if (KK <= 1) return i;
@@ -17,6 +18,7 @@
     return ((long)a * B + b) * KK + tap;
 }
 
+template <bool FOUR>
 __device__ __forceinline__ void fold_dw(const ud_wgrad_fold& f, int blk, double* smem) {
     double(*sm)[16][4] = reinterpret_cast<double(*)[16][4]>(smem);
     const int KK = f.p0 * f.p0, C = f.p1, KKC = KK * C, nparts = f.nparts;
@@ -26,7 +28,16 @@
     if (i < KKC) {
         const f32x4* p4 = reinterpret_cast<const f32x4*>(f.part + i);
         const long step = (long)KKC / 4;
-        for (int p = sl; p < nparts; p += 16) {
+        int p = sl;
+        if (FOUR) {
+            for (; p + 48 < nparts; p += 64) {
+                const f32x4 v0 = p4[(long)p * step], v1 = p4[(long)(p + 16) * step];
+                const f32x4 v2 = p4[(long)(p + 32) * step], v3 = p4[(long)(p + 48) * step];
+#pragma unroll
+                for (int e = 0; e < 4; ++e) v[e] += ((double)v0[e] + (double)v1[e]) + ((double)v2[e] + (double)v3[e]);
+            }
+        }
+        for (; p < nparts; p += 16) {
             const f32x4 w = p4[(long)p * step];
 #pragma unroll
             for (int e = 0; e < 4; ++e) v[e] += (double)w[e];
@@ -115,6 +126,20 @@
     if (f.dgamma) f.dgamma[c] = (float)b;
 }
 
+__device__ __forceinline__ void fold_gate(const ud_wgrad_fold& f, double* sm) {
+    double acc = 0.0;
+    for (int i = threadIdx.x; i < f.nparts; i += NT) acc += f.s1l[i];
+    acc = ud_wave_sum_d(acc);
+    if ((threadIdx.x & 63) == 0) sm[threadIdx.x >> 6] = acc;
+    __syncthreads();
+    if (threadIdx.x == 0) {
+        double tot = 0.0;
+        for (int i = 0; i < NT / 64; ++i) tot += sm[i];
+        const double a = 1.0 / (1.0 + exp(-(double)f.aux[0]));
+        f.dst[0] = (float)(tot * a * (1.0 - a));
+    }
+}
+
 __device__ __forceinline__ void fold_layout(const ud_wgrad_fold& f, int blk) {
     const int i = blk * NT + threadIdx.x;
     if (i < f.n) f.dst[out_index(i, f.p0, f.p1)] = f.part[i];
@@ -127,7 +152,9 @@
     const ud_wgrad_fold& f = a.it[j];
     const int blk = (int)blockIdx.x - a.block0[j];
     switch (f.kind) {
-        case UD_FOLD_DW: fold_dw(f, blk, sm); break;
+        case UD_FOLD_DW: fold_dw<false>(f, blk, sm); break;
+        case UD_FOLD_DW4: fold_dw<true>(f, blk, sm); break;
+        case UD_FOLD_GATE: fold_gate(f, sm); break;
         case UD_FOLD_F32: fold_f32(f, blk, sm); break;
         case UD_FOLD_PJ: fold_pj(f, blk, sm); break;
         case UD_FOLD_F64: fold_f64(f, blk, sm); break;
@@ -137,11 +164,14 @@
 }
 
 int item_blocks(const ud_wgrad_fold& f) {
-    if (!f.part || f.nparts < 1) return 0;
+    if (f.nparts < 1 || (!f.part && f.kind != UD_FOLD_GATE)) return 0;
     const bool conv = f.kind == UD_FOLD_F32 || f.kind == UD_FOLD_F64 || f.kind == UD_FOLD_LAYOUT;
     if (conv && f.p0 > 1 && (f.p1 < 1 || f.n < 1 || f.n % (f.p0 * f.p1))) return 0;
     switch (f.kind) {
+        case UD_FOLD_GATE:
+            return (f.dst && f.aux && f.s1l) ? 1 : 0;
         case UD_FOLD_DW:
+        case UD_FOLD_DW4:
             if (!f.dst || (f.p0 != 3 && f.p0 != 5) || f.p1 < 4 || f.p1 % 4 || f.p2 < 0 || f.p2 > 2 || (f.p2 != 0 && !f.aux)) return 0;
             return ud_cdiv(f.p0 * f.p0 * f.p1, 64);
         case UD_FOLD_F32:
diff --git a/unidefense_amd/kernels.py b/unidefense_amd/kernels.py
--- a/unidefense_amd/kernels.py
+++ b/unidefense_amd/kernels.py
@@ -2497,8 +2497,11 @@
     dspat = torch.empty_like(spat)
     dfreq = torch.empty_like(freq)
     dalpha = empty((), spat)
-    _call("ud_sfmix_bwd", _p(spat), _p(freq), _p(alpha), _p(dy), _p(dspat), _p(dfreq), _p(part), _p(dalpha), N, Ho,
+    defer = folds_deferred()
+    _call("ud_sfmix_bwd", _p(spat), _p(freq), _p(alpha), _p(dy), _p(dspat), _p(dfreq), _p(part), None if defer else _p(dalpha), N, Ho,
           Wo, Cc, int(pool), h, _stream())
+    if defer:
+        _defer_fold("gate", (dalpha,), keep=(part,), s1l=part.data_ptr(), aux=alpha, dst=dalpha, nparts=nb)
     return dspat, dfreq, dalpha
 
 
@@ -2516,8 +2519,11 @@
     dp = torch.empty_like(p)
     dq = torch.empty_like(p)
     dalpha = empty((), p)
-    _call("ud_gate_mix_bwd", _p(p), _p(q), _p(alpha), _p(dy), _p(dp), _p(dq), _p(part), _p(dalpha), p.numel(),
+    defer = folds_deferred()
+    _call("ud_gate_mix_bwd", _p(p), _p(q), _p(alpha), _p(dy), _p(dp), _p(dq), _p(part), None if defer else _p(dalpha), p.numel(),
           _stream())
+    if defer:
+        _defer_fold("gate", (dalpha,), keep=(part,), s1l=part.data_ptr(), aux=alpha, dst=dalpha, nparts=nb)
     return dp, dq, dalpha
 
 
@@ -2641,6 +2647,25 @@
     _call("ud_dynfilter_bwd", _p(dout2), _p(dmask_ext), _p(x2), _p(mask), C.c_void_p(argmax.data_ptr()), _p(w2),
           _p(dx), _p(dlogit), _p(dproj), M, Cproj, Cx, _stream())
     return dx, dlogit, dproj
+
+
+def dynfilter_bwd_w(dout2, dmask_ext, x2, mask, argmax, w2, Cproj, pre, nbias=0):
+    _chk(dout2, dmask_ext, x2, mask, w2, pre)
+    M, Cx = x2.shape
+    J = pre.shape[1]
+    dx = torch.empty_like(x2)
+    dlogit = empty((M,), x2)
+    dproj = empty((M, Cproj), x2)
+    blocks = _call("ud_dynfilter_bwd_blocks", M)
+    part = empty((blocks, J), x2)
+    g = empty((J,), x2)
+    gw, gb = g[:J - nbias], (g[J - nbias:] if nbias else None)
+    defer = folds_deferred()
+    _call("ud_dynfilter_bwd_w", _p(dout2), _p(dmask_ext), _p(x2), _p(mask), C.c_void_p(argmax.data_ptr()), _p(w2), _p(pre),
+          _p(dx), _p(dlogit), _p(dproj), _p(part), None if defer else _p(g), M, Cproj, Cx, J, _stream())
+    if defer:
+        _defer_fold("f64", (gw,) if gb is None else (gw, gb), part=part, dst=g, nparts=blocks, n=J)
+    return dx, dlogit, dproj, gw, gb
 
 
 _DFT_CACHE = {}
@@ -3439,8 +3464,12 @@
     chunks = max(1, min(N * Ho, -(-_DW_WGRAD_THREADS // lanes)))
     part = empty((chunks, K * K, Cc), x)
     dwt = empty((Cc, K * K), x)
-    _call("ud_dwconv_bwd_weight_ex", _p(x), _p(dy), _p(gate_alpha), int(gate_mode), _p(dwt), _p(part), chunks, N, H, W,
+    defer = folds_deferred()
+    _call("ud_dwconv_bwd_weight_ex", _p(x), _p(dy), _p(gate_alpha), int(gate_mode), None if defer else _p(dwt), _p(part), chunks, N, H, W,
           Cc, Ho, Wo, K, stride, pad_t, pad_l, h, _stream())
+    if defer:
+        _defer_fold("dw4", (dwt,), part=part, dst=dwt, aux=gate_alpha if gate_mode else None, nparts=chunks, p0=int(K), p1=int(Cc),
+                    p2=int(gate_mode) if gate_alpha is not None else 0)
     return dwt
 
 
@@ -3555,6 +3584,7 @@
     return dx
 
 
+MATERIALIZE_GRADS = False
 _WGRAD_FOLDS = None
 _WGRAD_PART_WS = Scratch(torch.float32)
 _FOLDS_IMMEDIATE = False
diff --git a/unidefense_amd/loss/pass_tail.py b/unidefense_amd/loss/pass_tail.py
--- a/unidefense_amd/loss/pass_tail.py
+++ b/unidefense_amd/loss/pass_tail.py
@@ -15,6 +15,7 @@
             return None if t is None else t.detach().contiguous()
         vals, grads = K.loss_tail(c(cls_out), tgt.contiguous(), n_real, n_fake, [c(f) for f in feats], c(fm), c(sm), c(spatial),
                                   c(freq), weights)
+        ctx.set_materialize_grads(K.MATERIALIZE_GRADS)
         ctx.grads = grads
         ctx.shapes = [None if t is None else t.shape for t in (cls_out, fm, sm, spatial, freq)]
         outs = vals.unbind(0)
@@ -24,6 +25,8 @@
     @staticmethod
     def backward(ctx, g, *_):
         grads = ctx.grads
+        if g is None:
+            return (None,) * (10 + sum(1 for k in grads if k.startswith("feat")))
         flat = grads["_flat"] * g
         base = grads["_flat"].data_ptr()
 
diff --git a/unidefense_amd/model/unidefense.py b/unidefense_amd/model/unidefense.py
--- a/unidefense_amd/model/unidefense.py
+++ b/unidefense_amd/model/unidefense.py
@@ -111,6 +111,7 @@
 class _NetFunction(torch.autograd.Function):
     @staticmethod
     def forward(ctx, model, x, noise_x, rng, *params):
+        ctx.set_materialize_grads(K.MATERIALIZE_GRADS)
         K.begin_forward(model)
         tape = T.Tape()
         if ctx.needs_input_grad[1] and noise_x is None:
diff --git a/unidefense_amd/tape.py b/unidefense_amd/tape.py
--- a/unidefense_amd/tape.py
+++ b/unidefense_amd/tape.py
@@ -715,20 +715,20 @@
                 return
             if dout is None:
                 dout = torch.zeros_like(out)
-            dx, dlogit, dproj = K.dynfilter_bwd(dout.view(-1, Cx), None if dmask is None else dmask.view(-1),
-                                                x2, mask, argmax, w2f, Cp)
+            args = (dout.view(-1, Cx), None if dmask is None else dmask.view(-1), x2, mask, argmax, w2f, Cp)
+            gw = gb = None
+            if _wgrad(tape):
+                dx, dlogit, dproj, gw, gb = K.dynfilter_bwd_w(*args, pre, 0 if b2 is None else 1)
+            else:
+                dx, dlogit, dproj = K.dynfilter_bwd(*args)
             tape.add_grad(x, dx.view(x.shape))
             tape.add_grad(proj, dproj.view(proj.shape))
             if diff_grad:
                 tape.add_grad(diff, K.outer(dlogit, w2f[2:2 + D]).view(diff.shape))
-            if not _wgrad(tape):
-                return
-            g = K.gemm_tn(dlogit.view(-1, 1), pre)
-            if b2 is None:
-                tape.add_param_grad(w2, g.view(w2.shape))
-            else:
-                tape.add_param_grad(w2, g[:, :-1].reshape(w2.shape))
-                tape.add_param_grad(b2, g[:, -1].reshape(b2.shape))
+            if gw is not None:
+                tape.add_param_grad(w2, gw)
+                if gb is not None:
+                    tape.add_param_grad(b2, gb)
         tape.record(bwd)
     return out, mask4
 
```

New measurement: 1506, median of 6. No clear change (+0.6%).
